# changzy00/pytorch-attention

Measured on AMD Instinct MI355X. Metric: forward images/sec through one step (+ ms/block), B=256 per GPU, 224x224-derived shapes, higher is better.
Workload: dtype f32/f16; 1 GPU; north-star step: C2 SE+CBAM+ECA, C3 ViT-Attn, C4 CSWin s1-4 + XCABlock + XCA, DA x2, Mixer, C5 ViT-Base fwd; B=256/GPU; precision=fp16-mfma, ranks_seen=1, gather=none (single rank), batch_per_gpu=256, parallelism=batch-shard x1, dist_backend=none, rccl_self_test=not run (single rank), distinct_gpus=1, full=off: --full adds calibration, roofline, per-block and CPU-baseline figures

## Files before the change

### include/mi355attn.h

```cpp
#ifndef MI355ATTN_H
#define MI355ATTN_H

#include <stddef.h>
#include <stdint.h>

#ifdef __cplusplus
extern "C" {
#endif

#define MI355_OK            0
#define MI355_EINVAL       -1
#define MI355_EUNSUPPORTED -2
#define MI355_EHIP         -3
#define MI355_ESYNC        -4
#define MI355_ERANGE (-5)

#define MI355_PREC_STRICT 0
#define MI355_PREC_FP16   1
#define MI355_PREC_BF16   2

#define MI355_ACT_NONE 0
#define MI355_ACT_GELU 1
#define MI355_ACT_RELU 2

// ... 88 lines not shown
};
size_t mi355_bam_workspace_bytes(int B, int C, int Cr, int H, int W);
int mi355_bam_fwd(const float* x, const float* const* params, float* y, int B, int C, int Cr, int H, int W, int dilation,
                  void* workspace, size_t workspace_bytes, mi355_stream_t stream);
int mi355_bam_gates_fwd(const float* x, const float* const* params, float* cg, float* sg, int B, int C, int Cr, int H, int W, int dilation,
                        void* workspace, size_t workspace_bytes, mi355_stream_t stream);
int mi355_zpool_fwd(const float* x, float* y, int B, int C, int H, int W, mi355_stream_t stream);
size_t mi355_attention_gate_workspace_bytes(int B, int H, int W);
int mi355_attention_gate_fwd(const float* x, const float* w, const float* affine, float* y, int B, int C, int H, int W, int ksize,
                             void* workspace, size_t workspace_bytes, mi355_stream_t stream);

enum {
    MI355_SK_CONV3_W = 0,
    MI355_SK_CONV3_SCALE,
    MI355_SK_CONV3_SHIFT,
    MI355_SK_CONV5_W,
    MI355_SK_CONV5_SCALE,
    MI355_SK_CONV5_SHIFT,
    MI355_SK_FC_W,
    MI355_SK_FC_B,
    MI355_SK_FC_BN_SCALE,
    MI355_SK_FC_BN_SHIFT,
    MI355_SK_FC1_W,
    MI355_SK_FC1_B,
    MI355_SK_FC2_W,
    MI355_SK_FC2_B,
    MI355_SK_NPARAMS
};
size_t mi355_sk_workspace_bytes(int B, int planes, int H, int W);
int mi355_sk_fwd(const float* x, const float* const* params, float* y, int B, int Cin, int planes, int groups, int d, int H, int W,
                 void* workspace, size_t workspace_bytes, mi355_stream_t stream);

size_t mi355_cam_workspace_bytes(int B, int C);
int mi355_cam_fwd(const float* x, const float* beta, float* y, int B, int C, int H, int W, int precision, void* workspace,
                  size_t workspace_bytes, mi355_stream_t stream);
int mi355_tokens_to_nchw_axpy_fwd(const float* tokens, const float* x, const float* alpha, float* y, int B, int HW, int C,
                                  mi355_stream_t stream);

int mi355_adaptive_pool_tokens_fwd(const float* x, float* y, int B, int H, int W, int C, int OH, int OW, mi355_stream_t stream);
int mi355_dwconv3x3_tokens_residual_fwd(const float* x, const float* weight, const float* bias, float* y, int B, int H, int W, int C,
                                        long y_batch_stride, mi355_stream_t stream);
int mi355_dwconv_nchw_tokens_fwd(const float* x, const float* weight, const float* bias, float* y, int B, int C, int H, int W, int ks,
                                 mi355_stream_t stream);
int mi355_qk_logits_fwd(const float* q, const float* k, float* logits, int B, int heads, int Nq, int Nkv, int head_dim, int ldq, int ldk,
                        int precision, mi355_stream_t stream);
int mi355_topk_mask_fwd(float* logits, long rows, int N, int k, mi355_stream_t stream);


int mi355_linear_fwd(const float* X, const float* W, const float* bias, const float* gamma, const float* resid,
                     float* Y, int M, int N, int K, int ldx, int ldy, int act, int precision,
                     mi355_stream_t stream);

int mi355_token_mix_fwd(const float* W, const float* X, const float* bias, const float* resid, float* Y,
                        int B, int T, int N, int C, int act, int precision, mi355_stream_t stream);

int mi355_layernorm_fwd(const float* x, const float* weight, const float* bias, float* y,
                        int rows, int cols, float eps, mi355_stream_t stream);

int mi355_cast16_fwd(const float* src, void* dst16, size_t n, int precision, mi355_stream_t stream);
int mi355_layernorm16_fwd(const float* x, const float* weight, const float* bias, void* y16, int rows, int cols, float eps,
                          int precision, mi355_stream_t stream);
int mi355_linear16_fwd(const void* X16, const void* W16, const float* bias, const float* gamma, const float* resid, void* Y,
                       int M, int N, int K, int ldx, int ldy, int act, int out16, int precision, mi355_stream_t stream);
size_t mi355_linear16_workspace_bytes(int M, int N, int K);
int mi355_linear16_x32_fwd(const float* X32, const void* W16, const float* bias, void* Y16, int M, int N, int K, int ldx, int ldy, int act,
                           int precision, mi355_stream_t stream);
int mi355_linear16_stats_fwd(const void* X16, const void* W16, const float* bias, const float* resid, float* Y, int M, int N, int K, int ldx,
                             int ldy, int precision, float* row_stats, float eps, mi355_stream_t stream);
int mi355_linear16_ln16_fwd(const void* X16, const void* W16, const float* bias, const float* resid, float* Y, const float* ln_w,
                            const float* ln_b, float eps, void* U16, int M, int N, int K, int ldx, int ldy, int ldu, int precision,
                            mi355_stream_t stream);
int mi355_linear16_ws_fwd(const void* X16, const void* W16, const float* bias, const float* gamma, const float* resid, void* Y,
                          int M, int N, int K, int ldx, int ldy, int act, int out16, int precision, void* ws, size_t ws_bytes,
                          mi355_stream_t stream);
int mi355_layernorm16_t_fwd(const float* x, const float* weight, const float* bias, void* ut16, int B, int N, int C, int NP, float eps,
                            int precision, mi355_stream_t stream);
int mi355_linear16_tr_fwd(const void* X16, const void* W16, const float* bias, const float* resid, float* Y, int M, int N, int K,
                          int ldx, int rows_per_image, int precision, mi355_stream_t stream);
size_t mi355_mixer_token_workspace_bytes(int B, int N, int C);
int mi355_mixer_token_fwd(const float* x, const float* ln_w, const float* ln_b, float ln_eps, const void* w1p16, const float* b1,
                          const void* w2s16, const float* b2, float* y, int B, int N, int C, int T, int precision, void* ws,
                          size_t ws_bytes, mi355_stream_t stream);
int mi355_ln_linear16_fwd(const float* X, const void* W16, const float* bias, void* Y, int M, int N, int K, int ldx, int ldy, float eps,
                          int act, int out16, int precision, mi355_stream_t stream);
int mi355_sdpa16_fwd(const void* qkv16, void* out16, int B, int N, int heads, int d, float scale, int precision,
                     mi355_stream_t stream);
int mi355_cswin_lepe_attn16_fwd(const void* qkv16, const float* getv_w, const float* getv_b, void* out16,
                                int B, int reso, int Ctot, int c0, int Cb, int heads, int Hsp, int Wsp,
                                float scale, int precision, mi355_stream_t stream);
int mi355_qkv_split16_fwd(const float* x, const void* w_hi, const void* w_lo, const void* w_v16, const float* bias, void* qkv5,
                          int M, int C, int K, int ldx, mi355_stream_t stream);
int mi355_sdpa16_split_fwd(const void* qkv5, void* out16, int B, int N, int heads, int d, float scale, mi355_stream_t stream);
int mi355_cswin_lepe_attn16_pair_fwd(const void* qkv16, const float* getv_w0, const float* getv_b0, const float* getv_w1,
                                     const float* getv_b1, void* out16, int B, int reso, int Ctot, int heads, int split, float scale,
                                     int precision, mi355_stream_t stream);

int mi355_proj_mlp_fused_fwd(const float* x, const void* ctx16, const void* wp16, const float* bp, const void* w1_16, const float* b1,
                             const void* w2_16, const float* b2, const float* gamma, float* y, long M, int C, int hidden, int layernorm,
                             float eps, int precision, mi355_stream_t stream);

int mi355_cswin_stripe_attn_fwd(const float* x, const void* wqkv16, const float* bqkv, const float* getv_w0, const float* getv_b0,
                                const float* getv_w1, const float* getv_b1, void* ctx16, int B, int reso, int C, int heads_per_branch,
                                int split, float scale, float eps, int precision, mi355_stream_t stream);

int mi355_mlp_fused_fwd(const float* x, const void* w1_16, const float* b1, const void* w2_16, const float* b2, const float* gamma,
                        float* y, long M, int C, int hidden, int layernorm, float eps, int precision, mi355_stream_t stream);


int mi355_sdpa_fwd(const float* qkv, float* out, int B, int N, int heads, int d, float scale, int precision,
                   mi355_stream_t stream);

int mi355_cswin_lepe_attn_fwd(const float* qkv, const float* getv_w, const float* getv_b, float* out,
                              int B, int reso, int Ctot, int c0, int Cb, int heads, int Hsp, int Wsp,
                              float scale, int precision, mi355_stream_t stream);

int mi355_xca_fwd(const float* qkv, const float* temperature, float* out, int B, int N, int heads, int d,
                  int precision, mi355_stream_t stream);
int mi355_xca16_fwd(const void* qkv, int qkv_is16, const float* temperature, void* out16, int B, int N, int heads, int d,
                    int precision, mi355_stream_t stream);

size_t mi355_lpi_workspace_bytes(int B, int H, int W, int C);
int    mi355_lpi_fwd(const float* x, const float* w1, const float* b1, const float* bn_w, const float* bn_b,
                     const float* bn_mean, const float* bn_var, float bn_eps, const float* w2, const float* b2,
                     const float* gamma, const float* resid, float* y, int B, int H, int W, int C,
                     void* ws, size_t ws_bytes, mi355_stream_t stream);
int    mi355_ln_lpi_fwd(const float* x, const float* ln_w, const float* ln_b, float ln_eps, const float* w1, const float* b1,
                        const float* bn_w, const float* bn_b, const float* bn_mean, const float* bn_var, float bn_eps, const float* w2,
                        const float* b2, const float* gamma, const float* resid, float* y, int B, int H, int W, int C, void* ws,
                        size_t ws_bytes, mi355_stream_t stream);

int mi355_patch_embed_fwd(const float* img, const float* Wp, const float* bp, const float* cls, const float* pos,
                          float* tokens, int B, int Cin, int H, int W, int ps, int E, int precision,
                          mi355_stream_t stream);
size_t mi355_patch_embed_workspace_bytes(int B, int Cin, int H, int W, int ps, int E, int precision);
int mi355_patch_embed_ws_fwd(const float* img, const float* Wp, const float* bp, const float* cls, const float* pos,
                             float* tokens, int B, int Cin, int H, int W, int ps, int E, int precision,
                             void* ws, size_t ws_bytes, mi355_stream_t stream);

size_t mi355_ln_fold_stats_bytes(int rows, int cols);
int mi355_ln_center16_fwd(const float* x, void* a16, float* rowtau, float* cvec, int rows, int cols, float eps, int precision,
                          mi355_stream_t stream);
int mi355_ln_finalize_fwd(const float* stats, const float* x, void* a16, float* cvec, float* rowtau, int rows, int cols, float eps,
                          float tol, int precision, unsigned* slow_rows, mi355_stream_t stream);
int mi355_linear16_emit_fwd(const void* X16, const void* W16, const float* bias, const float* resid, float* Y, int M, int N, int K, int ldx,
                            int act, int precision, const float* cvec, void* a16_out, float* stats, mi355_stream_t stream);
int mi355_linear16_lnfold_fwd(const void* A16, const void* W16, const float* bias, const float* rowtau, const float* colsum, void* Y16,
                              int M, int N, int K, int lda, int ldy, int act, int precision, mi355_stream_t stream);

size_t mi355_mhsa_workspace_bytes(int B, int N, int C, int x_is16);
int mi355_mhsa_fwd(const void* x, int x_is16, const void* Wqkv16, const float* b_qkv, const void* Wproj16, const float* b_proj,
                   const float* resid, float* y, int B, int N, int C, int heads, float scale, int precision, void* workspace,
                   size_t workspace_bytes, mi355_stream_t stream);

int mi355_sdpa_general_fwd(const void* q, const void* k, const void* v, const float* bias, void* out, int B, int num_heads, int Nq,
                           int Nkv, int head_dim, long ldq, long ldk, long ldv, long ldo, long bias_batch_stride, float scale,
                           int io16, int precision, mi355_stream_t stream);


int mi355_conv2d_tokens_fwd(const float* x, const float* weight, const float* bias, const float* pos, float* y, int B, int Cin,
                            int H, int W, int Cout, int KH, int KW, int stride, int pad, int ldw, int in_layout, int act,
                            int precision, mi355_stream_t stream);

int mi355_token_mean_fwd(const float* x, float* y, int B, int N, int C, long batch_stride, mi355_stream_t stream);

int mi355_class_attn_fwd(const float* q, const float* k, const float* v, float* out, int B, int N, int num_heads, int head_dim,
                         long ldq, long ldkv, float scale, mi355_stream_t stream);

int mi355_dwconv_patch_tokens_fwd(const float* x, const float* weight, const float* bias, float* y, int B, int H, int W, int C,
                                  int sr, mi355_stream_t stream);

int mi355_axpby_fwd(const float* x, const float* u, const float* gamma, float* y, long rows, int cols, long ldx, long ldu,
                    long ldy, float alpha, mi355_stream_t stream);

#define MI355_COMM_ID_BYTES 128
int    mi355_sdpa_core_fwd(const float* qkv, float* out, int B, int N, int heads, int d, float scale, int precision, mi355_stream_t stream);
size_t mi355_sdpa_core_workspace_bytes(int B, int N, int heads, int d);
int    mi355_gemm_bias_act_fwd(const float* X, const float* W, const float* bias, const float* gamma, const float* resid, float* Y, int M, int N,
                               int K, int ldx, int ldy, int act, int precision, mi355_stream_t stream);
size_t mi355_gemm_bias_act_workspace_bytes(int M, int N, int K);
int    mi355_mixer_token_mlp_fwd(const float* x, const float* ln_w, const float* ln_b, float ln_eps, const void* w1p16, const float* b1,
                                 const void* w2s16, const float* b2, float* y, int B, int N, int C, int T, int precision, void* ws,
                                 size_t ws_bytes, mi355_stream_t stream);
size_t mi355_mixer_token_mlp_workspace_bytes(int B, int N, int C);
size_t mi355_cswin_lepe_attn_workspace_bytes(int B, int reso, int Ctot);
size_t mi355_xca_workspace_bytes(int B, int N, int heads, int d);
size_t mi355_layernorm_workspace_bytes(int rows, int cols);

int mi355_ln_lpi_stats_fwd(const float* x, const float* stats, const float* ln_w, const float* ln_b, const float* w1, const float* b1,
                           const float* bn_w, const float* bn_b, const float* bn_mean, const float* bn_var, float bn_eps, const float* w2,
                           const float* b2, const float* gamma, const float* resid, float* y, int B, int H, int W, int C,
                           mi355_stream_t stream);

int mi355_comm_unique_id(void* id_out, size_t id_bytes);
int mi355_comm_init(const void* id, size_t id_bytes, int rank, int world, void** comm_out);
int mi355_allgather_f32(void* comm, const float* send, float* recv, size_t count, mi355_stream_t stream);
int mi355_comm_destroy(void* comm);

int mi355_bicubic_rows_fwd(const float* table, float* out, int n0h, int n0w, int oh, int ow, int dim, float scale_h, float scale_w,
                           mi355_stream_t stream);
int mi355_stream_copy(const void* src, void* dst, size_t bytes, mi355_stream_t stream);
int mi355_stream_read(const void* src, size_t bytes, float* sink, mi355_stream_t stream);
int mi355_mfma_yardstick(int shape, int iters, float* sink, unsigned long long* report, mi355_stream_t stream);
int mi355_event_time_begin(mi355_stream_t stream, void** handle);
int mi355_event_time_end(mi355_stream_t stream, void* handle, float* ms_out);

#ifdef __cplusplus
}
#endif
#endif
```

### pytorch-attention_amd/csrc/api.hip

```cpp
#include "common.h"
#include <atomic>
#include <cstring>
#include <mutex>
#include <algorithm>
#include <unordered_map>
#include <map>
#include <string>
#include <vector>

namespace mi355 {
static thread_local char g_err[512] = "";

constexpr int MAX_DEV = 64;
enum Opt { O_CHUNK_IMAGES, O_NT, O_REVERSE, O_GEMM_VARIANT, O_ECA_SINGLE, O_SE_SINGLE, O_CBAM_SINGLE, O_WS_PERSISTENT, O_STEM_DIRECT,
           O_ZOO_SINGLE, O_SPIN_LIMIT, O_GEMM_PA, O_GEMM_SPLITK, O_DA_FUSED, O_DA_RANGES, O_SE_OCC, O_LN_FOLD, O_GEMM_PA16, O_GEMM_PA_BLOCK, O_GEMM_PA_TAIL, O_LPI_PATCH, O_MIXER_FUSED, O_MIXER_EARLY, O_GEMM_SMALL, O_MLP_TT4, O_MIXER_STATS, O_ATTN_NW, O_GEMM_W4, O_RANGE_FALLBACK, O_GEMM_WREG, O_XCA_TR, O_MLP_WIDE, O_GEMM_WST, O_GEMM_WSLAB, O_IO16_OCC, O_COUNT };
struct OptDesc { const char* key; long def, lo, hi; };
static const OptDesc kOpts[O_COUNT] = {
    {"chunk_images", 0, 0, 1L << 40},
    {"nt", 3, 0, 3},
    {"reverse", 0, 0, 1},
    {"gemm_variant", 0, 0, 17},
    {"eca_single", 1, 0, 1},
    {"se_single", 1, 0, 1},
    {"cbam_single", 1, 0, 1},
    {"ws_persistent", 0, 0, 1},
    {"stem_direct", 1, 0, 1},
    {"zoo_single", 1, 0, 1},
    {"spin_limit", 1L << 22, 1024, 1L << 30},
    {"gemm_pa", 1, 0, 1},
    {"gemm_splitk", 1, 0, 1},
    {"da_fused", 1, 0, 1},
    {"da_ranges", 0, 0, 32},
    {"se_occ", 3, 2, 3},
    {"ln_fold", 0, 0, 1},
    {"gemm_pa16", 1, 0, 2},
    {"gemm_pa_block", 1, 0, 1},
    {"gemm_pa_tail", 10, 0, 100},
    {"lpi_patch", 1, 0, 1},
    {"mixer_fused", 1, 0, 1},
    {"mixer_early", 0, 0, 1},
    {"gemm_small", 1, 0, 1},
    {"mlp_tt4", 0, 0, 1},
    {"mixer_stats", 0, 0, 1},
    {"attn_nw", 8, 7, 8},
    {"gemm_w4", 1, 0, 1},
    {"range_fallback", 1, 0, 1},
    {"gemm_wreg", 1, 0, 1},
    {"xca_tr", 1, 0, 1},
    {"mlp_wide", 0, 0, 1},
    {"gemm_wst", 0, 0, 4},
    {"gemm_wslab", 1, 0, 2},
    {"io16_occ", 4, 2, 4},
};
static_assert(sizeof(kOpts) / sizeof(kOpts[0]) == O_COUNT, "one table row per option, in enum order");
namespace {
constexpr long OPT_UNSET = (long)0x8000000000000000ull;
struct OptBlock { std::atomic<long> v[O_COUNT]; };
OptBlock g_opt[MAX_DEV];
std::atomic<long> g_def[O_COUNT];
std::once_flag g_opt_once;
int cur_dev() {
    int dev = 0;
    if (hipGetDevice(&dev) != hipSuccess) { (void)hipGetLastError(); dev = 0; }
    return dev >= 0 && dev < MAX_DEV ? dev : 0;
}
void opt_init() {
    std::call_once(g_opt_once, [] {
        for (int i = 0; i < O_COUNT; ++i) g_def[i].store(kOpts[i].def, std::memory_order_relaxed);
        for (auto& b : g_opt)
            for (int i = 0; i < O_COUNT; ++i) b.v[i].store(OPT_UNSET, std::memory_order_relaxed);
    });
}
inline long opt(Opt o) {
    opt_init();
    const long v = g_opt[cur_dev()].v[o].load(std::memory_order_relaxed);
    return v != OPT_UNSET ? v : g_def[o].load(std::memory_order_relaxed);
}
}

char* err_buf() { return g_err; }

int fail(int code, const char* fmt, ...) {
    va_list ap;
    va_start(ap, fmt);
    vsnprintf(g_err, sizeof(g_err), fmt, ap);
    va_end(ap);
    return code;
}
long opt_chunk_images() { return opt(O_CHUNK_IMAGES); }
long opt_nt() { return opt(O_NT); }
long opt_reverse() { return opt(O_REVERSE); }
long opt_eca_single() { return opt(O_ECA_SINGLE); }
long opt_se_single() { return opt(O_SE_SINGLE); }
long opt_cbam_single() { return opt(O_CBAM_SINGLE); }
long opt_ws_persistent() { return opt(O_WS_PERSISTENT); }
long opt_ln_fold() { return opt(O_LN_FOLD); }
long opt_gemm_pa16() { return opt(O_GEMM_PA16); }
long opt_gemm_pa_block() { return opt(O_GEMM_PA_BLOCK); }
long opt_gemm_pa_tail() { return opt(O_GEMM_PA_TAIL); }
long opt_lpi_patch() { return opt(O_LPI_PATCH); }
long opt_mixer_early() { return opt(O_MIXER_EARLY); }
long opt_gemm_small() { return opt(O_GEMM_SMALL); }
long opt_mlp_tt4() { return opt(O_MLP_TT4); }
long opt_mixer_stats() { return opt(O_MIXER_STATS); }
long opt_attn_nw() { return opt(O_ATTN_NW); }
long opt_gemm_w4() { return opt(O_GEMM_W4); }
long opt_range_fallback() { return opt(O_RANGE_FALLBACK); }
long opt_gemm_wreg() { return opt(O_GEMM_WREG); }
long opt_xca_tr() { return opt(O_XCA_TR); }
long opt_mlp_wide() { return opt(O_MLP_WIDE); }
long opt_gemm_wst() { return opt(O_GEMM_WST); }
long opt_gemm_wslab() { return opt(O_GEMM_WSLAB); }

namespace {
struct WsEntry { unsigned long long key; };
std::mutex g_ws_mu;
std::unordered_map<const void*, WsEntry> g_ws;
}

bool stream_is_capturing(hipStream_t st) {
    hipStreamCaptureStatus cs = hipStreamCaptureStatusNone;
    if (hipStreamIsCapturing(st, &cs) != hipSuccess) {
        (void)hipGetLastError();
        return false;
    }
    return cs != hipStreamCaptureStatusNone;
}

bool ws_known(const void* region, unsigned long long key, hipStream_t st) {
    if (!opt_ws_persistent()) return false;
    std::lock_guard<std::mutex> lk(g_ws_mu);
    auto it = g_ws.find(region);
    if (it != g_ws.end() && it->second.key == key) return true;
    if (!stream_is_capturing(st)) g_ws[region] = WsEntry{key};
    return false;
}
namespace {
__global__ __launch_bounds__(256) void ws_zero_kernel(unsigned* p, size_t words) {
    for (size_t i = (size_t)blockIdx.x * 256 + threadIdx.x; i < words; i += (size_t)gridDim.x * 256) p[i] = 0u;
}
}
hipError_t ws_zero_async(void* p, size_t bytes, hipStream_t st) {
    const size_t words = bytes / 4;
    if (!words) return hipSuccess;
    size_t blocks = (words + 1023) / 1024;
    if (blocks > 2048) blocks = 2048;
    ws_zero_kernel<<<(int)blocks, 256, 0, st>>>(static_cast<unsigned*>(p), words);
    return hipGetLastError();
}
void ws_forget(const void* region) {
    std::lock_guard<std::mutex> lk(g_ws_mu);
    g_ws.erase(region);
}
void ws_forget_range(const void* base, size_t bytes) {
    std::lock_guard<std::mutex> lk(g_ws_mu);
    const char* lo = static_cast<const char*>(base);
    for (auto it = g_ws.begin(); it != g_ws.end();) {
        const char* p = static_cast<const char*>(it->first);
        if (p >= lo && p < lo + bytes) it = g_ws.erase(it);
        else ++it;
    }
}

namespace {
constexpr int THREAD_SLOTS = 64;
constexpr size_t SLOT_WORDS = 16 * MAX_DEV;
std::once_flag g_sync_once;
unsigned* g_sync_block = nullptr;
std::mutex g_slot_mu;
bool g_slot_used[THREAD_SLOTS] = {};
struct ThreadSlot {
    int idx = -1;
    ~ThreadSlot() {
        if (idx < 0 || idx >= THREAD_SLOTS) return;
        std::lock_guard<std::mutex> lk(g_slot_mu);
        g_slot_used[idx] = false;
    }
};
thread_local ThreadSlot t_slot;
unsigned* thread_words() {
    if (!g_sync_block) return nullptr;
    if (t_slot.idx < 0) {
        std::lock_guard<std::mutex> lk(g_slot_mu);
        int i = 0;
        while (i < THREAD_SLOTS && g_slot_used[i]) ++i;
        if (i < THREAD_SLOTS) {
            g_slot_used[i] = true;
            std::memset(g_sync_block + i * SLOT_WORDS, 0, SLOT_WORDS * sizeof(unsigned));
        }
        t_slot.idx = i;
    }
    return g_sync_block + t_slot.idx * SLOT_WORDS + 16 * cur_dev();
}
}
unsigned* sync_err_word() {
    std::call_once(g_sync_once, [] {
        const size_t bytes = (THREAD_SLOTS + 1) * SLOT_WORDS * sizeof(unsigned);
        void* p = nullptr;
        if (hipHostMalloc(&p, bytes, hipHostMallocMapped | hipHostMallocCoherent | hipHostMallocPortable) == hipSuccess && p) {
            std::memset(p, 0, bytes);
            g_sync_block = static_cast<unsigned*>(p);
        } else {
            (void)hipGetLastError();
        }
    });
    return thread_words();
}
unsigned* sync_err_word_on(hipStream_t st) {
    if (!g_sync_block && stream_is_capturing(st)) return nullptr;
    return sync_err_word();
}
namespace {
struct RangeMark {
    int armed = 0, dirty = 0, fresh = 0, have = 0, count = 0, expect = 0;
    hipEvent_t ev = nullptr;
    hipStream_t st = nullptr;
};
std::mutex g_ev_mu;
std::vector<hipEvent_t> g_ev_pool[MAX_DEV];
struct ThreadMarks {
    RangeMark m[MAX_DEV];
    ~ThreadMarks() {
        std::lock_guard<std::mutex> lk(g_ev_mu);
        for (int d = 0; d < MAX_DEV; ++d)
            if (m[d].ev) g_ev_pool[d].push_back(m[d].ev);
    }
};
thread_local ThreadMarks t_marks;
RangeMark& rmark(int dev) { return t_marks.m[dev]; }
void range_mark_record(RangeMark& m, int dev) {
    m.dirty = 0;
    if (stream_is_capturing(m.st)) return;
    if (!m.ev) {
        {
            std::lock_guard<std::mutex> lk(g_ev_mu);
            if (!g_ev_pool[dev].empty()) { m.ev = g_ev_pool[dev].back(); g_ev_pool[dev].pop_back(); }
        }
        if (!m.ev && hipEventCreateWithFlags(&m.ev, hipEventDisableTiming) != hipSuccess) { (void)hipGetLastError(); m.ev = nullptr; return; }
    }
    if (hipEventRecord(m.ev, m.st) == hipSuccess) m.have = 1;
    else (void)hipGetLastError();
}
}
void range_mark_before_launch() {
    const int dev = cur_dev();
    RangeMark& m = rmark(dev);
    if (!m.dirty || m.fresh) return;
    if (m.expect > 0 && m.count >= m.expect) range_mark_record(m, dev);
}
void range_mark_entry_done() {
    RangeMark& m = rmark(cur_dev());
    if (!m.fresh) return;
    m.fresh = 0;
    m.dirty = 1;
}
unsigned* range_word(hipStream_t st) {
    if (!g_sync_block && stream_is_capturing(st)) return nullptr;
    unsigned* w = sync_err_word();
    if (w) {
        RangeMark& m = rmark(cur_dev());
        if (m.armed) {
            m.st = st;
            ++m.count;
            m.fresh = 1;
        }
// ... 277 lines not shown
```

### pytorch-attention_amd/csrc/attn.hip

```cpp
#include "common.h"
#include "mma.h"
#include "bufops.h"
#include <type_traits>

namespace {

struct AttnArgs {
    const void* qkv;
    void* out;
    const float* lepe_w;
    const float* lepe_b;
    int L, Ctot, c0, heads;
    int koff, voff, oc0;
    int reso, Hsp, Wsp, nWx, nwin;
    int T;
    unsigned wsp_magic;
    float scale;
    int pre_scale;
};

struct AttnPair {
    AttnArgs a0, a1;
    int split;
};
struct AttnPairRg : AttnPair {
    unsigned* ovf;
};
template <bool IO16>
using attn_kargs = typename std::conditional<IO16, AttnPair, AttnPairRg>::type;
template <bool IO16>
const attn_kargs<IO16>& attn_pick(const AttnPairRg& p) { return p; }

#ifndef MI355_ATTN_FMA_SM
#define MI355_ATTN_FMA_SM 1
#endif
template <int PREC, int D, int KT, bool LEPE, bool IO16, int NW, int OCC = 1, int TFULL = -1>
__global__ __launch_bounds__(NW * 64, OCC) void win_attn_kernel(const attn_kargs<IO16> pr) {
    constexpr bool FMA_SM = MI355_ATTN_FMA_SM != 0;
    const int lid = xcd_contiguous_block();
    const bool second = lid >= pr.split;
    const AttnArgs a = second ? pr.a1 : pr.a0;
    constexpr int NTHR = NW * 64;
    static_assert(!IO16 || PREC != 0, "16-bit I/O exists for the fp16 / bf16 operand modes only");
    using M_ = Mma<PREC>;
    using v8 = typename M_::v8;
    using v4 = typename M_::v4;
    using el = typename M_::e;
    constexpr int NS = M_::NSPLIT;
    constexpr int TK = KT * 16;
    constexpr int KP = D + 8;
    constexpr int VP = TK + 4;
    constexpr bool RG = !IO16 && PREC == 1;
    float rgm = 0.f;
    constexpr int OP = IO16 ? D + 8 : D + 4;
    constexpr int K_EL = TK * KP, V_EL = D * VP;
    using slab_t = typename std::conditional<IO16, unsigned short, float>::type;
    __shared__ __attribute__((aligned(16))) unsigned short s_k[NS * K_EL];
    __shared__ __attribute__((aligned(16))) unsigned short s_v[NS * V_EL];
    __shared__ __attribute__((aligned(16))) slab_t s_o[NW * 16 * OP];

    const int t = threadIdx.x, lane = t & 63, wave = t >> 6;
    int bid = lid - (second ? pr.split : 0);
    const int head = bid % a.heads; bid /= a.heads;
    const int win = bid % a.nwin;
    const int b = bid / a.nwin;
    const int T = a.T;
    const int wy0 = (win / a.nWx) * a.Hsp, wx0 = (win % a.nWx) * a.Wsp;
    const int ch0 = a.c0 + head * D;
    const int och0 = a.oc0 + head * D;
    const long row3 = 3L * a.Ctot;
    using gel = typename std::conditional<IO16, el, float>::type;
    const gel* base = static_cast<const gel*>(a.qkv) + (long)b * a.L * row3 + ch0;
    auto srow = [&](int s) { return a.Wsp == 1 ? s : (int)__umulhi((unsigned)s, a.wsp_magic); };
    auto tok = [&](int s) { const int r = srow(s); return (wy0 + r) * a.reso + wx0 + (s - r * a.Wsp); };

    const int l15 = lane & 15, g = lane >> 4;
    const int nqt = (T + 15) >> 4;
    constexpr int NQ = (KT + NW - 1) / NW;
    const rsrc_t img_rs = make_rsrc(IO16 ? static_cast<const void*>(base) : nullptr, IO16 ? (bufops_u32)((long)a.L * row3 * sizeof(gel)) : 0u);
    auto ld16 = [&](bool live, int token, int el_off) -> v8 {
        const bufops_u32 off = live ? (bufops_u32)((token * (int)row3 + el_off) * 2) : OOB;
        return __builtin_bit_cast(v8, __builtin_amdgcn_raw_buffer_load_b128(img_rs, off, 0, 0));
    };
    v8 qraw[IO16 ? NQ : 1][D / 32];
    if constexpr (IO16) {
#pragma unroll
        for (int iq = 0; iq < NQ; ++iq) {
            const int qs = (wave + iq * NW) * 16 + l15;
            const int tq = tok(qs < T ? qs : 0);
#pragma unroll
            for (int ks = 0; ks < D / 32; ++ks) qraw[iq][ks] = ld16(qs < T, tq, ks * 32 + g * 8);
        }
    }
    __shared__ float s_lw[LEPE ? D * 10 : 1];
    if constexpr (LEPE) {
        for (int q = t; q < D * 10; q += NTHR) {
            const int c = q / 10, i = q - c * 10;
            s_lw[q] = i < 9 ? a.lepe_w[(long)(head * D + c) * 9 + i] : a.lepe_b[head * D + c];
        }
    }

    constexpr int D4 = D / 4;
    if constexpr (IO16) {
        constexpr int D8 = D / 8;
        constexpr int NKI = (TK * D8 + NTHR - 1) / NTHR, NVI = ((TK / 4) * D8 + NTHR - 1) / NTHR;
        v8 kreg[NKI];
        v8 vreg[NVI][4];
#pragma unroll
        for (int it = 0; it < NKI; ++it) {
            const int idx = t + it * NTHR, key = idx / D8, d8 = idx % D8;
            const bool live = idx < TK * D8 && key < T;
            kreg[it] = ld16(live, tok(live ? key : 0), a.koff + d8 * 8);
        }
#pragma unroll
        for (int it = 0; it < NVI; ++it) {
            const int idx = t + it * NTHR, kg = idx / D8, d8 = idx % D8;
#pragma unroll
            for (int j = 0; j < 4; ++j) {
                const int key = kg * 4 + j;
                const bool live = idx < (TK / 4) * D8 && key < T;
                vreg[it][j] = ld16(live, tok(live ? key : 0), a.voff + d8 * 8);
            }
        }
#pragma unroll
        for (int it = 0; it < NKI; ++it) {
            const int idx = t + it * NTHR, key = idx / D8, d8 = idx % D8;
            if (idx < TK * D8) *reinterpret_cast<v8*>(s_k + key * KP + d8 * 8) = kreg[it];
        }
#pragma unroll
        for (int it = 0; it < NVI; ++it) {
            const int idx = t + it * NTHR, kg = idx / D8, d8 = idx % D8;
            if (idx < (TK / 4) * D8) {
#pragma unroll
                for (int q = 0; q < 8; ++q)
                    *reinterpret_cast<v4*>(s_v + (d8 * 8 + q) * VP + kg * 4) =
                        v4{vreg[it][0][q], vreg[it][1][q], vreg[it][2][q], vreg[it][3][q]};
            }
        }
    } else {
    for (int idx = t; idx < TK * D4; idx += NTHR) {
        const int key = idx / D4, d4 = idx % D4;
        f4 v = {0.f, 0.f, 0.f, 0.f};
        if (key < T) v = *reinterpret_cast<const f4*>(base + (long)tok(key) * row3 + a.koff + d4 * 4);
        if constexpr (RG) rgm = rg_absmax4(rgm, v);
        const v4 h = M_::cvt(v);
        *reinterpret_cast<v4*>(s_k + key * KP + d4 * 4) = h;
        if constexpr (NS == 2) *reinterpret_cast<v4*>(s_k + K_EL + key * KP + d4 * 4) = M_::cvt_lo(v, h);
    }
    for (int idx = t; idx < (TK / 4) * D4; idx += NTHR) {
        const int kg = idx / D4, d4 = idx % D4;
        f4 r[4];
#pragma unroll
        for (int j = 0; j < 4; ++j) {
            const int key = kg * 4 + j;
            r[j] = f4{0.f, 0.f, 0.f, 0.f};
            if (key < T) r[j] = *reinterpret_cast<const f4*>(base + (long)tok(key) * row3 + a.voff + d4 * 4);
            if constexpr (RG) rgm = rg_absmax4(rgm, r[j]);
        }
        const f4 c[4] = {{r[0].x, r[1].x, r[2].x, r[3].x}, {r[0].y, r[1].y, r[2].y, r[3].y},
                         {r[0].z, r[1].z, r[2].z, r[3].z}, {r[0].w, r[1].w, r[2].w, r[3].w}};
#pragma unroll
        for (int q = 0; q < 4; ++q) {
            const v4 h = M_::cvt(c[q]);
            *reinterpret_cast<v4*>(s_v + (d4 * 4 + q) * VP + kg * 4) = h;
            if constexpr (NS == 2) *reinterpret_cast<v4*>(s_v + V_EL + (d4 * 4 + q) * VP + kg * 4) = M_::cvt_lo(c[q], h);
        }
    }
    }
    __shared__ unsigned short s_tap[LEPE ? TK * 9 : 1];
    if constexpr (LEPE) {
        for (int q = t; q < NS * D; q += NTHR) s_v[(q / D) * V_EL + (q % D) * VP + TK] = 0;
        for (int q = t; q < T * 9; q += NTHR) {
            const int slot = q / 9, tap = q - slot * 9;
            const int ty = srow(slot), tx = slot - ty * a.Wsp;
            const int yy = ty + tap / 3 - 1, xx = tx + tap % 3 - 1;
            s_tap[q] = (unsigned short)(((yy >= 0 && yy < a.Hsp && xx >= 0 && xx < a.Wsp) ? yy * a.Wsp + xx : TK) * 2);
        }
    }
    __syncthreads();

    slab_t* slab = s_o + wave * 16 * OP;
#pragma unroll
    for (int iq = 0; iq < NQ; ++iq) {
        const int qt = wave + iq * NW;
        if (qt >= nqt) break;
        const int qs = qt * 16 + l15;
        v8 qf[D / 32][NS];
        {
            const gel* qrow = base + (long)tok(qs < T ? qs : 0) * row3;
#pragma unroll
            for (int ks = 0; ks < D / 32; ++ks) {
                f4 lo4 = {0.f, 0.f, 0.f, 0.f}, hi4 = {0.f, 0.f, 0.f, 0.f};
                if constexpr (IO16) {
                    const v8 raw = qraw[iq][ks];
                    if (!a.pre_scale) { qf[ks][0] = raw; continue; }
                    lo4 = f4{(float)raw[0], (float)raw[1], (float)raw[2], (float)raw[3]};
                    hi4 = f4{(float)raw[4], (float)raw[5], (float)raw[6], (float)raw[7]};
                } else if (qs < T) {
                    lo4 = *reinterpret_cast<const f4*>(qrow + ks * 32 + g * 8);
                    hi4 = *reinterpret_cast<const f4*>(qrow + ks * 32 + g * 8 + 4);
                }
                if (a.pre_scale) { lo4 = lo4 * a.scale; hi4 = hi4 * a.scale; }
                if constexpr (RG) rgm = rg_absmax4(rg_absmax4(rgm, lo4), hi4);
                const v4 h0 = M_::cvt(lo4), h1 = M_::cvt(hi4);
                qf[ks][0] = v8{h0.x, h0.y, h0.z, h0.w, h1.x, h1.y, h1.z, h1.w};
                if constexpr (NS == 2) {
                    const v4 e0 = M_::cvt_lo(lo4, h0), e1 = M_::cvt_lo(hi4, h1);
                    qf[ks][1] = v8{e0.x, e0.y, e0.z, e0.w, e1.x, e1.y, e1.z, e1.w};
                }
            }
        }
        f4 o[D / 16];
        float sum;
        const f4 zero4 = {0.f, 0.f, 0.f, 0.f};
        f4 s[KT];
#pragma unroll
        for (int kt = 0; kt < KT; ++kt) {
            f4 acc = zero4;
            if (kt < TFULL || kt * 16 < T) {
#pragma unroll
                for (int ks = 0; ks < D / 32; ++ks) {
                    v8 kf[NS];
#pragma unroll
                    for (int sp = 0; sp < NS; ++sp)
                        kf[sp] = *reinterpret_cast<const v8*>(s_k + sp * K_EL + (kt * 16 + l15) * KP + ks * 32 + g * 8);
                    acc = mma_step<PREC>(kf, qf[ks], acc);
                }
            }
            s[kt] = acc;
        }
        const float post = (a.pre_scale ? 1.0f : a.scale) * 1.44269504088896340736f;
        float m = -INFINITY;
        sum = 0.f;
        if constexpr (PREC != 0 && FMA_SM) {
#pragma unroll
            for (int kt = 0; kt < KT; ++kt)
#pragma unroll
                for (int r = 0; r < 4; ++r) {
                    const int key = kt * 16 + g * 4 + r;
                    const float v = (kt < TFULL || key < T) ? s[kt][r] : -INFINITY;
                    s[kt][r] = v;
                    m = fmaxf(m, v);
                }
            m = fmaxf(m, __shfl_xor(m, 16, WAVE));
            m = fmaxf(m, __shfl_xor(m, 32, WAVE));
            const float mneg = -(m * post);
#pragma unroll
            for (int kt = 0; kt < KT; ++kt)
#pragma unroll
                for (int r = 0; r < 4; ++r) {
                    s[kt][r] = __builtin_amdgcn_exp2f(__builtin_fmaf(s[kt][r], post, mneg));
                }
        } else {
#pragma unroll
            for (int kt = 0; kt < KT; ++kt)
#pragma unroll
                for (int r = 0; r < 4; ++r) {
                    const int key = kt * 16 + g * 4 + r;
                    const float v = (kt < TFULL || key < T) ? s[kt][r] * post : -INFINITY;
                    s[kt][r] = v;
                    m = fmaxf(m, v);
                }
            m = fmaxf(m, __shfl_xor(m, 16, WAVE));
            m = fmaxf(m, __shfl_xor(m, 32, WAVE));
#pragma unroll
            for (int kt = 0; kt < KT; ++kt)
#pragma unroll
                for (int r = 0; r < 4; ++r) {
                    const float p = __builtin_amdgcn_exp2f(s[kt][r] - m);
                    s[kt][r] = p;
                    sum += p;
                }
        }
        if constexpr (!(PREC != 0 && FMA_SM)) {
            sum += __shfl_xor(sum, 16, WAVE);
            sum += __shfl_xor(sum, 32, WAVE);
        }
#pragma unroll
        for (int nt = 0; nt < D / 16; ++nt) o[nt] = zero4;
        f4 osum = zero4;
        typedef typename M_::e el1_t;
        const v8 ones = v8{(el1_t)1.0f, (el1_t)1.0f, (el1_t)1.0f, (el1_t)1.0f, (el1_t)1.0f, (el1_t)1.0f, (el1_t)1.0f, (el1_t)1.0f};
#pragma unroll
        for (int kb = 0; kb < KT / 2; ++kb) {
            if (2 * kb < TFULL || kb * 32 < T) {
                v8 pf[NS];
                {
                    const f4 p0 = s[2 * kb], p1 = s[2 * kb + 1];
                    const v4 h0 = M_::cvt(p0), h1 = M_::cvt(p1);
                    pf[0] = v8{h0.x, h0.y, h0.z, h0.w, h1.x, h1.y, h1.z, h1.w};
                    if constexpr (NS == 2) {
                        const v4 e0 = M_::cvt_lo(p0, h0), e1 = M_::cvt_lo(p1, h1);
                        pf[1] = v8{e0.x, e0.y, e0.z, e0.w, e1.x, e1.y, e1.z, e1.w};
                    }
                }
#pragma unroll
                for (int nt = 0; nt < D / 16; ++nt) {
                    v8 vf[NS];
#pragma unroll
                    for (int sp = 0; sp < NS; ++sp) {
                        const unsigned short* vr = s_v + sp * V_EL + (nt * 16 + l15) * VP + kb * 32 + g * 4;
                        const v4 a0 = *reinterpret_cast<const v4*>(vr);
                        const v4 a1 = *reinterpret_cast<const v4*>(vr + 16);
                        vf[sp] = v8{a0.x, a0.y, a0.z, a0.w, a1.x, a1.y, a1.z, a1.w};
                    }
                    o[nt] = mma_step<PREC>(vf, pf, o[nt]);
                }
                if constexpr (PREC != 0 && FMA_SM) osum = M_::mma(ones, pf[0], osum);
            }
        }
        if constexpr (PREC != 0 && FMA_SM) sum = osum.x;
        const float inv = __builtin_amdgcn_rcpf(sum);
        int off[LEPE ? 9 : 1];
        bool qlive = false;
        if constexpr (LEPE) {
            const int qslot = qt * 16 + l15;
            qlive = qslot < T;
            const unsigned short* tp = s_tap + (qlive ? qslot : 0) * 9;
#pragma unroll
            for (int i = 0; i < 9; ++i) off[i] = tp[i];
        }
#pragma unroll
        for (int nt = 0; nt < D / 16; ++nt) {
            f4 val = o[nt] * inv;
            if constexpr (LEPE) {
                if (qlive) {
#pragma unroll
                    for (int r = 0; r < 4; ++r) {
                        const int d = nt * 16 + g * 4 + r;
                        const float* lwp = s_lw + d * 10;
                        const char* vrow = reinterpret_cast<const char*>(s_v + d * VP);
                        float acc = lwp[9];
#pragma unroll
                        for (int i = 0; i < 9; ++i) {
                            float vv = (float)(*reinterpret_cast<const el*>(vrow + off[i]));
                            if constexpr (NS == 2) vv += (float)(*reinterpret_cast<const el*>(vrow + V_EL * 2 + off[i]));
                            acc = __builtin_fmaf(lwp[i], vv, acc);
                        }
                        val[r] += acc;
                    }
                }
            }
            if constexpr (IO16) *reinterpret_cast<v4*>(slab + l15 * OP + nt * 16 + g * 4) = M_::cvt(val);
            else *reinterpret_cast<f4*>(slab + l15 * OP + nt * 16 + g * 4) = val;
        }
        __builtin_amdgcn_wave_barrier();
        __builtin_amdgcn_fence(__ATOMIC_ACQ_REL, "wavefront");
        if constexpr (IO16) {
            constexpr int LPR = D / 8, RPI = 64 / LPR;
#pragma unroll
            for (int it = 0; it < 16 / RPI; ++it) {
                const int r = it * RPI + lane / LPR, c8 = (lane % LPR) * 8;
                const int qslot = qt * 16 + r;
                if (qslot < T)
                    *reinterpret_cast<v8*>(static_cast<gel*>(a.out) + ((long)b * a.L + tok(qslot)) * a.Ctot + och0 + c8) =
                        *reinterpret_cast<const v8*>(slab + r * OP + c8);
            }
        } else {
            constexpr int LPR = D / 4, RPI = 64 / LPR;
#pragma unroll
            for (int it = 0; it < 16 / RPI; ++it) {
                const int r = it * RPI + lane / LPR, c4 = (lane % LPR) * 4;
                const int qslot = qt * 16 + r;
                if (qslot < T)
                    *reinterpret_cast<f4*>(static_cast<gel*>(a.out) + ((long)b * a.L + tok(qslot)) * a.Ctot + och0 + c4) =
                        *reinterpret_cast<const f4*>(slab + r * OP + c4);
            }
        }
        __builtin_amdgcn_wave_barrier();
        __builtin_amdgcn_fence(__ATOMIC_ACQ_REL, "wavefront");
    }
    if constexpr (RG) rg_report(rgm, pr.ovf, 7u);
}

template <int D, bool LEPE, bool IO16>
int launch_attn(const AttnArgs& a, int B, int precision, hipStream_t st, const AttnArgs* other = nullptr) {
    AttnPairRg pr{};
    pr.a0 = a;
    pr.split = B * a.nwin * a.heads;
    int grid = pr.split;
    if (other) {
        pr.a1 = *other;
        grid += B * other->nwin * other->heads;
    }
    if (IO16 && precision == MI355_PREC_STRICT)
        return mi355::fail(MI355_EINVAL, "16-bit activation I/O needs precision 1 (fp16) or 2 (bf16)");
    if (!IO16 && precision == MI355_PREC_FP16) pr.ovf = mi355::range_word(st);
    MI355_TRACE(st, "win_attn_kernel<d=%d%s%s> B=%d windows=%d heads=%d tokens=%d", D, LEPE ? ",lepe" : "", IO16 ? ",io16" : "", B, a.nwin, a.heads, a.T);
#define GO(P, KT_, NW_) win_attn_kernel<P, D, KT_, LEPE, (IO16 && P != 0), NW_><<<grid, NW_ * 64, 0, st>>>(attn_pick<(IO16 && P != 0)>(pr))
#define GO_OCC(P, KT_, NW_, OCC_) win_attn_kernel<P, D, KT_, LEPE, (IO16 && P != 0), NW_, ((IO16 && P != 0 && D == 32) ? OCC_ : 1)><<<grid, NW_ * 64, 0, st>>>(attn_pick<(IO16 && P != 0)>(pr))
#define GO_FULL(P, KT_, NW_, OCC_, TF_) \
    win_attn_kernel<P, D, KT_, LEPE, (IO16 && P != 0), NW_, ((IO16 && P != 0 && D == 32) ? OCC_ : 1), TF_><<<grid, NW_ * 64, 0, st>>>(attn_pick<(IO16 && P != 0)>(pr))
    const bool hot = IO16 && (!other || other->T == a.T);
#define BYKT(P)                                          \
    do {                                                 \
        if (a.T <= 64) { if (hot && P != 0 && a.T >= 48) GO_FULL(P, 4, 4, 6, 3); else GO_OCC(P, 4, 4, 6); }          \
        else if (a.T <= 128) { if (hot && P != 0 && a.T >= 96) GO_FULL(P, 8, 4, 5, 6); else GO_OCC(P, 8, 4, 5); }    \
        else if (IO16 && P != 0) {                                                                                    \
             \
                                \
            if (a.T >= 192 && a.T <= 208 && mi355::opt_attn_nw() == 7) GO_FULL(P, 14, 7, 1, 12);                          \
            else if (a.T >= 192) GO_FULL(P, 14, 8, 1, 12); else GO(P, 14, 8); }                                          \
        else GO(P, 14, 4);                               \
    } while (0)
    switch (precision) {
        case MI355_PREC_STRICT: BYKT(0); break;
        case MI355_PREC_FP16:   BYKT(1); break;
        case MI355_PREC_BF16:   BYKT(2); break;
        default: return mi355::fail(MI355_EINVAL, "precision must be 0, 1 or 2 (got %d)", precision);
    }
#undef BYKT
#undef GO_FULL
#undef GO_OCC
#undef GO
    return MI355_OK;
}

}

static int sdpa_common(const void* qkv, void* out, int B, int N, int heads, int d, float scale, int precision, bool io16,
                       hipStream_t st) {
    AttnArgs a{};
    a.qkv = qkv; a.out = out; a.L = N; a.Ctot = heads * d; a.c0 = 0; a.heads = heads;
    a.koff = a.Ctot; a.voff = 2 * a.Ctot; a.oc0 = 0;
    a.reso = N; a.Hsp = 1; a.Wsp = N; a.nWx = 1; a.nwin = 1; a.T = N; a.scale = scale; a.pre_scale = 0;
    a.wsp_magic = (unsigned)(((1ull << 32) + (unsigned)N - 1) / (unsigned)N);
    if (d == 64) return io16 ? launch_attn<64, false, true>(a, B, precision, st) : launch_attn<64, false, false>(a, B, precision, st);
    return io16 ? launch_attn<32, false, true>(a, B, precision, st) : launch_attn<32, false, false>(a, B, precision, st);
}

static AttnArgs lepe_args(const void* qkv, const float* getv_w, const float* getv_b, void* out, int reso, int Ctot, int c0, int heads,
                          int Hsp, int Wsp, float scale) {
    AttnArgs a{};
    a.qkv = qkv; a.out = out; a.lepe_w = getv_w; a.lepe_b = getv_b;
    a.L = reso * reso; a.Ctot = Ctot; a.c0 = c0; a.heads = heads;
    a.koff = Ctot; a.voff = 2 * Ctot; a.oc0 = c0;
    a.reso = reso; a.Hsp = Hsp; a.Wsp = Wsp; a.nWx = reso / Wsp; a.nwin = (reso / Hsp) * (reso / Wsp); a.T = Hsp * Wsp;
    a.scale = scale; a.pre_scale = 1;
    a.wsp_magic = (unsigned)(((1ull << 32) + (unsigned)Wsp - 1) / (unsigned)Wsp);
    return a;
}

static int lepe_common(const void* qkv, const float* getv_w, const float* getv_b, void* out, int B, int reso, int Ctot, int c0, int Cb,
                       int heads, int Hsp, int Wsp, float scale, int precision, bool io16, hipStream_t st) {
    (void)Cb;
    const AttnArgs a = lepe_args(qkv, getv_w, getv_b, out, reso, Ctot, c0, heads, Hsp, Wsp, scale);
    return io16 ? launch_attn<32, true, true>(a, B, precision, st) : launch_attn<32, true, false>(a, B, precision, st);
}

#define SDPA_CHECKS(fn)                                                                                                   \
    MI355_CHECK_ARG(qkv && out && B > 0 && N > 0 && heads > 0);                                                           \
    if (!(d == 32 || d == 64)) return mi355::fail(MI355_EUNSUPPORTED, fn ": head dim %d (built: 32, 64)", d);            \
    if (N > 224) return mi355::fail(MI355_EUNSUPPORTED, fn ": sequence length %d > 224 (single-pass softmax core)", N);   \
    MI355_CHECK_ARG(aligned16(qkv) && aligned16(out))

#define LEPE_CHECKS(fn)                                                                                                    \
    MI355_CHECK_ARG(qkv && getv_w && getv_b && out);                                                                       \
    MI355_CHECK_ARG(B > 0 && reso > 0 && Ctot > 0 && c0 >= 0 && Cb > 0 && c0 + Cb <= Ctot && heads > 0 && Cb % heads == 0); \
    MI355_CHECK_ARG(Hsp > 0 && Wsp > 0 && reso % Hsp == 0 && reso % Wsp == 0);                                             \
    if (Cb / heads != 32) return mi355::fail(MI355_EUNSUPPORTED, fn ": head dim %d (built: 32)", Cb / heads);             \
    if (Hsp * Wsp > 224) return mi355::fail(MI355_EUNSUPPORTED, fn ": %d tokens per stripe window > 224", Hsp * Wsp);     \
    MI355_CHECK_ARG((Ctot & 7) == 0 && (c0 & 7) == 0 && aligned16(qkv) && aligned16(out))

extern "C" {

int mi355_sdpa_fwd(const float* qkv, float* out, int B, int N, int heads, int d, float scale, int precision,
                   mi355_stream_t stream) {
    SDPA_CHECKS("mi355_sdpa_fwd");
    int rc = sdpa_common(qkv, out, B, N, heads, d, scale, precision, false, static_cast<hipStream_t>(stream));
    if (rc) return rc;
    MI355_LAUNCH_CHECK();
    return MI355_OK;
}

int mi355_sdpa16_fwd(const void* qkv, void* out, int B, int N, int heads, int d, float scale, int precision,
                     mi355_stream_t stream) {
    SDPA_CHECKS("mi355_sdpa16_fwd");
    int rc = sdpa_common(qkv, out, B, N, heads, d, scale, precision, true, static_cast<hipStream_t>(stream));
    if (rc) return rc;
    MI355_LAUNCH_CHECK();
    return MI355_OK;
}

int mi355_cswin_lepe_attn_fwd(const float* qkv, const float* getv_w, const float* getv_b, float* out, int B, int reso, int Ctot,
                              int c0, int Cb, int heads, int Hsp, int Wsp, float scale, int precision, mi355_stream_t stream) {
    LEPE_CHECKS("mi355_cswin_lepe_attn_fwd");
    int rc = lepe_common(qkv, getv_w, getv_b, out, B, reso, Ctot, c0, Cb, heads, Hsp, Wsp, scale, precision, false,
                         static_cast<hipStream_t>(stream));
    if (rc) return rc;
    MI355_LAUNCH_CHECK();
    return MI355_OK;
}

int mi355_cswin_lepe_attn16_pair_fwd(const void* qkv, const float* getv_w0, const float* getv_b0, const float* getv_w1, const float* getv_b1,
                                     void* out, int B, int reso, int Ctot, int heads, int split, float scale, int precision,
                                     mi355_stream_t stream) {
    MI355_CHECK_ARG(qkv && getv_w0 && getv_b0 && getv_w1 && getv_b1 && out);
    MI355_CHECK_ARG(B > 0 && reso > 0 && Ctot > 0 && heads > 0 && (Ctot / 2) % heads == 0 && split > 0 && reso % split == 0);
    if (Ctot / 2 / heads != 32) return mi355::fail(MI355_EUNSUPPORTED, "mi355_cswin_lepe_attn16_pair_fwd: head dim %d (built: 32)", Ctot / 2 / heads);
    if (reso * split > 224) return mi355::fail(MI355_EUNSUPPORTED, "mi355_cswin_lepe_attn16_pair_fwd: %d tokens per stripe window > 224", reso * split);
    MI355_CHECK_ARG((Ctot & 15) == 0 && aligned16(qkv) && aligned16(out));
    const AttnArgs a0 = lepe_args(qkv, getv_w0, getv_b0, out, reso, Ctot, 0, heads, reso, split, scale);
    const AttnArgs a1 = lepe_args(qkv, getv_w1, getv_b1, out, reso, Ctot, Ctot / 2, heads, split, reso, scale);
    int rc = launch_attn<32, true, true>(a0, B, precision, static_cast<hipStream_t>(stream), &a1);
    if (rc) return rc;
    MI355_LAUNCH_CHECK();
    return MI355_OK;
}

int mi355_cswin_lepe_attn16_fwd(const void* qkv, const float* getv_w, const float* getv_b, void* out, int B, int reso, int Ctot,
                                int c0, int Cb, int heads, int Hsp, int Wsp, float scale, int precision, mi355_stream_t stream) {
    LEPE_CHECKS("mi355_cswin_lepe_attn16_fwd");
    int rc = lepe_common(qkv, getv_w, getv_b, out, B, reso, Ctot, c0, Cb, heads, Hsp, Wsp, scale, precision, true,
                         static_cast<hipStream_t>(stream));
    if (rc) return rc;
    MI355_LAUNCH_CHECK();
    return MI355_OK;
}

}
```

### pytorch-attention_amd/csrc/common.h

```cpp
#pragma once
#include <hip/hip_runtime.h>
#include <cstdarg>
#include <cstdio>
#include <cstdint>
#include "../../include/mi355attn.h"

#define MI355_ABI_VERSION 1
#define WAVE 64

namespace mi355 {
char* err_buf();
int   fail(int code, const char* fmt, ...);
long  opt_chunk_images();
long  opt_nt();
long  opt_reverse();
long  opt_gemm_variant();
long  opt_gemm_splitk();
long  opt_gemm_pa();
long  opt_da_fused();
long  opt_da_ranges();
long  opt_eca_single();
long  opt_se_single();
long  opt_se_occ();
long  opt_io16_occ();
long  opt_ws_persistent();
long  opt_ln_fold();
long  opt_gemm_pa16();
long  opt_gemm_pa_block();
long  opt_gemm_pa_tail();
long  opt_lpi_patch();
long  opt_mixer_early();
long  opt_gemm_small();
long  opt_mlp_tt4();
long  opt_mixer_stats();
long  opt_attn_nw();
long  opt_gemm_w4();
long  opt_gemm_wreg();
long  opt_xca_tr();
long  opt_mlp_wide();
long  opt_gemm_wst();
long  opt_gemm_wslab();
bool  mlp_wide_applicable(int C, int hidden);
int   mlp_wide(const float* x, const void* w1_16, const float* b1, const void* w2_16, const float* b2, const float* gamma, float* y, long M, int C,
               int layernorm, float eps, int precision, hipStream_t st);
int   gemm_small_nt(const float* A, const float* B, const float* bias, float* C, int M, int N, int K, int lda, int ldb, int ldc, int precision,
                    hipStream_t st);
void  ws_forget(const void* region);
bool  ws_known(const void* region, unsigned long long key, hipStream_t st);
hipError_t ws_zero_async(void* p, size_t bytes, hipStream_t st);
unsigned* sync_err_word_on(hipStream_t st);
bool  stream_is_capturing(hipStream_t st);
void  ws_forget_range(const void* base, size_t bytes);
long  opt_cbam_single();
unsigned* sync_err_word();
unsigned* range_word(hipStream_t st);
int   range_pending(const char* who);
void  range_mark_before_launch();
void  range_mark_entry_done();
int   range_arm(int on);
int   range_wait();
long  range_launches();
unsigned  spin_limit();
int   sync_pending(const char* who);
int   resident_slots(int per_cu);
bool  trace_on();
int   trace_begin();
long  trace_end(char* buf, size_t n);
struct TraceScope {
    int idx;
    hipStream_t st;
    TraceScope(hipStream_t st_, const char* fmt, ...);
    ~TraceScope();
    TraceScope(const TraceScope&) = delete;
    TraceScope& operator=(const TraceScope&) = delete;
};
#define MI355_TRACE(st, ...) mi355::TraceScope trace_scope_(st, __VA_ARGS__)
int   func_dynamic_lds(const void* fn, int bytes);
long  opt_zoo_single();
long  opt_stem_direct();
bool  stem_conv_applicable(int Cin, int Cout, int KH, int KW, int in_layout, const float* bias, const float* pos, const float* y);
int   stem_conv(const float* x, const float* w, const float* bias, const float* pos, float* y, int B, int Cin, int H, int W, int Cout, int KH,
                int KW, int stride, int pad, int ldw, int in_layout, int act, hipStream_t st);
size_t zoo_workspace_bytes(int B, int C);
size_t cbam_single_extra_bytes(int B, int C, int H, int W);
bool  cbam_single_applicable(int C, int Cr, int H, int W, int ks);
int   cbam_single(const float* x, const float* w1, const float* w2, const float* wconv, float* y, int B, int C, int Cr, int H, int W,
                  int ks, void* extra, hipStream_t st);
size_t se_single_extra_bytes(int B, int C);
bool  se_single_applicable(int C, int Cr, int H, int W);
struct SeExtra {
    const float* b1;
    const float* b2;
    int gate;
};
int   se_single(const float* x, const float* w1, const float* w2, float* y, int B, int C, int Cr, int H, int W, void* state,
                void* gran, SeExtra ex, hipStream_t st);
bool  eca_single_applicable(int C, int k, int H, int W);
int   eca_single(const float* x, const float* taps, float* y, int B, int C, int k, int H, int W, hipStream_t st);
size_t fused_state_bytes(int B);
bool   double_attn_fused_ok(int B, int C, int cm, int cn, int HW, int precision);
size_t double_attn_fused_workspace(int B, int C, int HW);
int    double_attn_fused(const float* x, const float* wA, const float* bA, const float* wB, const float* bB, const float* wV, const float* bV,
                         const float* wP, const float* bP, float* y, int B, int C, int HW, int precision, void* ws, hipStream_t st);
bool   double_attn_small_ok(int B, int C, int cm, int cn, int HW, int precision);
int    double_attn_small(const float* x, const float* wA, const float* bA, const float* wB, const float* bB, const float* wV, const float* bV,
                         const float* wP, const float* bP, float* y, int B, int C, int HW, int precision, hipStream_t st);
int gemm_nt(const float* A, const float* B, const float* bias, const float* gamma, const float* resid, float* C, int M, int N,
            int K, int lda, int ldb, int ldc, int act, int precision, hipStream_t st);
int gemm_nt_batched(const float* A, const float* B, float* C, int batch, int M, int N, int K, int lda, int ldb, int ldc, long sA,
                    long sB, long sC, int precision, hipStream_t st);
int gemm_kn_batched(const float* A, const float* B, const float* bias_row, const float* resid, float* C, int batch, int M,
                    int N, int K, int lda, int ldb, int ldc, long sA, long sB, long sC, int act, int precision,
                    hipStream_t st);
}

#define MI355_CHECK_ARG(cond)                                                                   \
    do {                                                                                        \
        if (!(cond)) return mi355::fail(MI355_EINVAL, "%s: invalid argument: %s", __func__, #cond); \
    } while (0)

#define MI355_HIP(call)                                                                         \
    do {                                                                                        \
        hipError_t e_ = (call);                                                                 \
        if (e_ != hipSuccess)                                                                   \
            return mi355::fail(MI355_EHIP, "%s: %s -> %s", __func__, #call, hipGetErrorString(e_)); \
    } while (0)

#define MI355_LAUNCH_CHECK()                                                                    \
    do {                                                                                        \
        hipError_t e_ = hipGetLastError();                                                      \
        if (e_ != hipSuccess)                                                                   \
            return mi355::fail(MI355_EHIP, "%s: kernel launch -> %s", __func__, hipGetErrorString(e_)); \
        mi355::range_mark_entry_done();                                                         \
    } while (0)

static inline bool aligned16(const void* p) { return (reinterpret_cast<uintptr_t>(p) & 15u) == 0; }
static inline int  cdiv(long a, long b) { return (int)((a + b - 1) / b); }

#if defined(__HIPCC__)
__device__ __forceinline__ float wave_sum(float v) {
#pragma unroll
    for (int o = 32; o > 0; o >>= 1) v += __shfl_xor(v, o, WAVE);
    return v;
}
__device__ __forceinline__ float wave_max(float v) {
#pragma unroll
    for (int o = 32; o > 0; o >>= 1) v = fmaxf(v, __shfl_xor(v, o, WAVE));
    return v;
}
template <int XOR> __device__ __forceinline__ float swz_xor(float v) {
    return __builtin_bit_cast(float, __builtin_amdgcn_ds_swizzle(__builtin_bit_cast(int, v), (XOR << 10) | 0x1f));
}
__device__ __forceinline__ float wave_sum_sw(float v) {
    float a = v, b = v;
    asm volatile("s_nop 1\n\tv_permlane32_swap_b32 %0, %1\n\ts_nop 1" : "+v"(a), "+v"(b));
    v = a + b;
    v += swz_xor<16>(v);
    v += swz_xor<8>(v);
    v += swz_xor<4>(v);
    v += swz_xor<2>(v);
    v += swz_xor<1>(v);
    return v;
}

__device__ __forceinline__ int xcd_contiguous_block() {
    const int nwg = gridDim.x, orig = blockIdx.x, xcd = orig & 7, q = nwg >> 3, r = nwg & 7;
    return (xcd < r ? xcd * (q + 1) : r * (q + 1) + (xcd - r) * q) + (orig >> 3);
}
__device__ __forceinline__ float relu_nan(float v) {
    const float r = fmaxf(v, 0.f);
    return ((__float_as_uint(v) & 0x7fffffffu) > 0x7f800000u) ? v : r;
}
__device__ __forceinline__ float sigmoidf_(float z) { return 1.0f / (1.0f + expf(-z)); }
typedef float rg_f4 __attribute__((ext_vector_type(4)));
__device__ __forceinline__ float rg_fold(float m, float g) {
    const int u = (int)(__float_as_uint(g) + 0x00800000u);
    const int mi = (int)__float_as_uint(m);
    return __uint_as_float((unsigned)(u > mi ? u : mi));
}
__device__ __forceinline__ float rg_absmax4(float m, rg_f4 v) {
    return rg_fold(m, fmaxf(fmaxf(fabsf(v.x), fabsf(v.y)), fmaxf(fabsf(v.z), fabsf(v.w))));
}
__device__ __forceinline__ float rg_absmax1(float m, float v) { return rg_fold(m, fabsf(v)); }
__device__ __forceinline__ void rg_report(float m, unsigned* word, unsigned code) {
    if (word && (int)__float_as_uint(m) >= (int)(0x477FF000u + 0x00800000u))
        __hip_atomic_store(word, code, __ATOMIC_RELAXED, __HIP_MEMORY_SCOPE_SYSTEM);
}
__device__ __forceinline__ float rg_absmax4_f(float m, rg_f4 v) {
    const float g = fmaxf(fmaxf(fabsf(v.x), fabsf(v.y)), fmaxf(fabsf(v.z), fabsf(v.w)));
    return g < __builtin_inff() ? fmaxf(m, g) : m;
}
__device__ __forceinline__ void rg_report_f(float m, unsigned* word, unsigned code) {
    if (word && m >= 65520.0f) __hip_atomic_store(word, code, __ATOMIC_RELAXED, __HIP_MEMORY_SCOPE_SYSTEM);
}
// ... 85 lines not shown
```

### pytorch-attention_amd/csrc/gemm16.h

```cpp
#pragma once
#include "common.h"
#include "mma.h"

namespace g16 {

constexpr int BK = 64;

struct G16Args {
    const void* A; const void* B; void* C;
    const float* bias; const float* gamma; const float* resid;
    int M, N, K, lda, ldb, ldc;
    int act;
    int tr_rows;
    int resid_period;
    unsigned* ovf;
    const float* Af;
    float ln_eps;
    void* lnc_a; int lnc_lda; float* lnc_stats; const float* lnc_c;
    const float* rowtau; const float* colsum;
    float* row_stats;
    void* ln16_out; const float* ln16_w; const float* ln16_b; int ln16_ld;
};

template <typename T> struct Vec8;
template <> struct Vec8<_Float16> { using t = h8; using t4 = h4; };
template <> struct Vec8<__bf16> { using t = b8; using t4 = b4; };

template <typename T>
__device__ __forceinline__ f4 mma16(typename Vec8<T>::t a, typename Vec8<T>::t b, f4 c);
template <>
__device__ __forceinline__ f4 mma16<_Float16>(h8 a, h8 b, f4 c) { return __builtin_amdgcn_mfma_f32_16x16x32_f16(a, b, c, 0, 0, 0); }
template <>
__device__ __forceinline__ f4 mma16<__bf16>(b8 a, b8 b, f4 c) { return __builtin_amdgcn_mfma_f32_16x16x32_bf16(a, b, c, 0, 0, 0); }

}

namespace mi355 {
int gemm16_p8(const g16::G16Args& g, int out16, int precision, void* ws, size_t ws_bytes, hipStream_t st);
size_t gemm16_p8_workspace_bytes(int M, int N, int K);
int gemm16_pa(const g16::G16Args& g, int out16, int precision, hipStream_t st, int abl = 0);
int gemm16_w4(const g16::G16Args& g, int out16, int precision, hipStream_t st);
int gemm16_wreg(const g16::G16Args& g, int out16, int precision, hipStream_t st);
int gemm16_wst(const g16::G16Args& g, int out16, int precision, hipStream_t st);
int gemm16_wslab(const g16::G16Args& g, int out16, int precision, hipStream_t st);
int gemm16_wslab_check(const g16::G16Args& g, int precision);
int linear16_dispatch(const g16::G16Args& g, int out16, int precision, void* ws, size_t ws_bytes, hipStream_t st);
}
```

### pytorch-attention_amd/csrc/gemm16.hip

```cpp
#include <type_traits>
#include "gemm16.h"

namespace {
using namespace g16;

template <typename T, bool OUT16, int BM, int BN, int WM, int WN, bool PRIO, int STAGES, bool TR = false>
__global__ __launch_bounds__(WM * WN * 64) void gemm16_kernel(const G16Args g) {
    using v8 = typename Vec8<T>::t;
    using v4 = typename Vec8<T>::t4;
    constexpr int NW = WM * WN;
    constexpr int TM = BM / WM, TN = BN / WN, MF = TM / 16, NF = TN / 16;
    constexpr int STAGE = (BM + BN) * BK;
    constexpr int IA = BM / 8 / NW, IB = BN / 8 / NW;
    constexpr int LDS_BYTES = STAGES * STAGE * 2;
    static_assert(BM % (8 * NW) == 0 && BN % (8 * NW) == 0 && TM % 32 == 0 && TN % 16 == 0, "tile/wave geometry");
    __shared__ __attribute__((aligned(16))) unsigned char lds_raw[LDS_BYTES];
    T* lds = reinterpret_cast<T*>(lds_raw);

    const int t = threadIdx.x, lane = t & 63, wave = t >> 6;
    const int wr = wave / WN, wc = wave % WN;
    const int tiles_n = (g.N + BN - 1) / BN;
    int wg;
    {
        const int nwg = gridDim.x, bid = blockIdx.x, xcd = bid & 7, q = nwg >> 3, r = nwg & 7;
// ... 439 lines not shown
    const int rc2 = mi355::gemm16_wslab(g, 1, precision, st);
    if (rc2 != MI355_OK) return rc2;
    MI355_LAUNCH_CHECK();
    return MI355_OK;
}

int mi355_linear16_ws_fwd(const void* X16, const void* W16, const float* bias, const float* gamma, const float* resid, void* Y, int M,
                          int N, int K, int ldx, int ldy, int act, int out16, int precision, void* ws, size_t ws_bytes,
                          mi355_stream_t stream) {
    MI355_CHECK_ARG(X16 && W16 && Y && M > 0 && N > 0 && K > 0 && ldx >= K && ldy >= N);
    MI355_CHECK_ARG(act == MI355_ACT_NONE || act == MI355_ACT_GELU);
    MI355_CHECK_ARG(precision == MI355_PREC_FP16 || precision == MI355_PREC_BF16);
    if ((K % BK) || (N & 3) || (ldx & 7) || (ldy & 3) || !aligned16(X16) || !aligned16(W16) || !aligned16(Y) ||
        (bias && !aligned16(bias)) || (gamma && !aligned16(gamma)) || (resid && !aligned16(resid)))
        return mi355::fail(MI355_EUNSUPPORTED, "mi355_linear16_fwd: needs K %% 64 == 0, N %% 4 == 0, 16-byte aligned rows (K=%d N=%d ldx=%d)",
                           K, N, ldx);
    G16Args g{};
    g.A = X16; g.B = W16; g.C = Y; g.bias = bias; g.gamma = gamma; g.resid = resid;
    g.M = M; g.N = N; g.K = K; g.lda = ldx; g.ldb = K; g.ldc = ldy; g.act = act;
    if (out16 && precision == MI355_PREC_FP16) g.ovf = mi355::range_word(static_cast<hipStream_t>(stream));
    return mi355::linear16_dispatch(g, out16, precision, ws, ws_bytes, static_cast<hipStream_t>(stream));
}

int mi355_linear16_stats_fwd(const void* X16, const void* W16, const float* bias, const float* resid, float* Y, int M, int N, int K, int ldx,
                             int ldy, int precision, float* row_stats, float eps, mi355_stream_t stream) {
    MI355_CHECK_ARG(X16 && W16 && resid && Y && row_stats && M > 0 && N > 0 && K > 0 && ldx >= K && ldy >= N);
    MI355_CHECK_ARG(precision == MI355_PREC_FP16 || precision == MI355_PREC_BF16);
    G16Args g{};
    g.row_stats = row_stats; g.ln_eps = eps;
    if (const int rc = linear16_wreg_fwd(g, X16, W16, bias, resid, Y, M, N, K, ldx, ldy, precision, static_cast<hipStream_t>(stream),
                                         "mi355_linear16_stats_fwd", "and a statistics pass"))
        return rc;
    MI355_LAUNCH_CHECK();
    return MI355_OK;
}

int mi355_linear16_ln16_fwd(const void* X16, const void* W16, const float* bias, const float* resid, float* Y, const float* ln_w,
                            const float* ln_b, float eps, void* U16, int M, int N, int K, int ldx, int ldy, int ldu, int precision,
                            mi355_stream_t stream) {
    MI355_CHECK_ARG(X16 && W16 && resid && Y && ln_w && ln_b && U16 && M > 0 && N > 0 && K > 0 && ldx >= K && ldy >= N && ldu >= N);
    MI355_CHECK_ARG(precision == MI355_PREC_FP16 || precision == MI355_PREC_BF16);
    G16Args g{};
    g.ln16_out = U16; g.ln16_w = ln_w; g.ln16_b = ln_b; g.ln16_ld = ldu; g.ln_eps = eps;
    if (const int rc = linear16_wreg_fwd(g, X16, W16, bias, resid, Y, M, N, K, ldx, ldy, precision, static_cast<hipStream_t>(stream),
                                         "mi355_linear16_ln16_fwd", "+ mi355_layernorm16_fwd"))
        return rc;
    MI355_LAUNCH_CHECK();
    return MI355_OK;
}

}

int mi355::linear16_dispatch(const G16Args& g, int out16, int precision, void* ws, size_t ws_bytes, hipStream_t st) {
    const int M = g.M, N = g.N, K = g.K;
    if (g.resid_period && (K == 64 || K == 128 || out16 || !g.resid)) return MI355_EUNSUPPORTED;
    const struct { long variant, wst, wslab, pa, pa16, pa_tail, wreg, w4; } opt = {
        mi355::opt_gemm_variant(), mi355::opt_gemm_wst(), mi355::opt_gemm_wslab(), mi355::opt_gemm_pa(), mi355::opt_gemm_pa16(),
        mi355::opt_gemm_pa_tail(), mi355::opt_gemm_wreg(), mi355::opt_gemm_w4()};
    const int ncu = mi355::resident_slots(1);
    const bool gelu = g.act == MI355_ACT_GELU;
    long variant = opt.variant;
    if (variant >= 15) {
        static const char* const what[] = {"persistent kernel",
                                           "the two-accumulator kernel",
                                           "the one-wave-per-SIMD kernel"};
        const int rc = variant == 15 ? mi355::gemm16_p8(g, out16, precision, ws, ws_bytes, st)
                     : variant == 16 ? mi355::gemm16_pa(g, out16, precision, st) : mi355::gemm16_w4(g, out16, precision, st);
        if (rc == MI355_EUNSUPPORTED) return mi355::fail(rc, "mi355_linear16_fwd: %s does not take this shape", what[variant - 15]);
        return checked(rc);
    }
    if (variant == 0) {
        int rc;
        if ((opt.wst == 2 || opt.wst == 4 || ((opt.wst & 1) && g.act == MI355_ACT_NONE)) &&
            (rc = checked(mi355::gemm16_wst(g, out16, precision, st))) != MI355_EUNSUPPORTED)
            return rc;
        if ((K == 64 || K == 128) && M >= 2048 && (!out16 || (N & 7) == 0)) {
            MI355_TRACE(st, "gemm16_ws_kernel<%s> M=%d N=%d K=%d", out16 ? "out16" : "out32", M, N, K);
            launch_ws<false>(g, out16, precision, K == 64 ? 2 : 1, ncu, st);
            MI355_LAUNCH_CHECK();
            return MI355_OK;
        }
        if ((opt.wslab == 2 || (opt.wslab == 1 && (gelu || (M & 255)))) &&
            (rc = checked(mi355::gemm16_wslab(g, out16, precision, st))) != MI355_EUNSUPPORTED)
            return rc;
        const long pa_tiles = (N & 255) ? (long)(M / 256) * (N / 128) : (long)cdiv(M, 128) * (N / 256);
        const bool pa_fills = 2 * pa_tiles >= ncu;
        if (out16 && opt.pa && pa_fills && (K <= 512 || (opt.pa16 >= 1 && gelu) || opt.pa16 >= 2) &&
            (rc = checked(mi355::gemm16_pa(g, out16, precision, st))) != MI355_EUNSUPPORTED)
            return rc;
        if (opt.wreg && (rc = checked(mi355::gemm16_wreg(g, out16, precision, st))) != MI355_EUNSUPPORTED) return rc;
        if (!out16 && (g.resid || N <= 768) && opt.pa && pa_fills) {
            const int bmt = (N & 255) ? 256 : 128, tn = (N & 255) ? N / 128 : N / 256;
            const long left = pa_tiles % ncu;
            if (opt.pa_tail > 0 && pa_tiles > ncu && left > 0 && left * 100 <= opt.pa_tail * ncu && K >= 1024 && M % bmt == 0 &&
                !g.resid_period && !g.lnc_a) {
                const int rows1 = (int)((pa_tiles - left) / tn) * bmt, rows2 = M - rows1;
                G16Args g1 = g, g2 = g;
                g1.M = rows1;
                g2.M = rows2;
                g2.A = static_cast<const char*>(g.A) + (size_t)rows1 * g.lda * 2;
                g2.C = static_cast<char*>(g.C) + (size_t)rows1 * g.ldc * 4;
                if (g.resid) g2.resid = g.resid + (size_t)rows1 * g.ldc;
                rc = mi355::gemm16_pa(g1, out16, precision, st);
                if (rc == MI355_OK) {
                    MI355_LAUNCH_CHECK();
                    const int grid = cdiv(rows2, 32) * cdiv(N, 64);
                    MI355_TRACE(st, "gemm16_kernel<tail 32x64> M=%d N=%d K=%d", rows2, N, K);
                    if (precision == MI355_PREC_FP16) gemm16_kernel<_Float16, false, 32, 64, 1, 4, false, 10><<<grid, 256, 0, st>>>(g2);
                    else                              gemm16_kernel<__bf16, false, 32, 64, 1, 4, false, 10><<<grid, 256, 0, st>>>(g2);
                    MI355_LAUNCH_CHECK();
                    return MI355_OK;
                }
                if (rc != MI355_EUNSUPPORTED) return rc;
            }
            if ((rc = checked(mi355::gemm16_pa(g, out16, precision, st))) != MI355_EUNSUPPORTED) return rc;
        }
        if ((long)cdiv(M, 256) * cdiv(N, 256) >= ncu && K >= 256) {
            if (out16 && K >= 576 && K < 1536 && opt.w4 && (rc = checked(mi355::gemm16_w4(g, out16, precision, st))) != MI355_EUNSUPPORTED)
                return rc;
            if ((rc = checked(mi355::gemm16_p8(g, out16, precision, ws, ws_bytes, st))) != MI355_EUNSUPPORTED) return rc;
        }
        variant = (N <= 64) ? 9 : (N < 256 ? 1 : 7);
        if (variant == 7 && (long)cdiv(M, 128) * cdiv(N, 256) < ncu) variant = 1;
    }
    else if (variant == 8) variant = 0;
    MI355_TRACE(st, "gemm16_kernel<variant %ld,%s> M=%d N=%d K=%d%s", variant, out16 ? "out16" : "out32", M, N, K, gelu ? " gelu" : "");
#define LAUNCH(T_, O_, BM_, BN_, WM_, WN_, P_, S_)                                                         \
    gemm16_kernel<T_, O_, BM_, BN_, WM_, WN_, P_, S_><<<cdiv(M, BM_) * cdiv(N, BN_), WM_ * WN_ * 64, 0, st>>>(g)
#define BY_VARIANT(T_, O_)                                                 \
    do {                                                                   \
        switch (variant) {                                                 \
            case 1: LAUNCH(T_, O_, 128, 128, 2, 2, true, 2); break;        \
            case 2: LAUNCH(T_, O_, 256, 128, 4, 2, false, 2); break;       \
            case 3: LAUNCH(T_, O_, 256, 256, 2, 4, false, 2); break;       \
            case 4: LAUNCH(T_, O_, 256, 256, 2, 4, true, 2); break;        \
            case 5: LAUNCH(T_, O_, 128, 128, 2, 2, true, 1); break;        \
            case 6: LAUNCH(T_, O_, 256, 128, 4, 2, true, 1); break;        \
            case 7: LAUNCH(T_, O_, 128, 256, 2, 4, true, 1); break;        \
            case 9: LAUNCH(T_, O_, 256, 64, 4, 1, true, 1); break;         \
            default: LAUNCH(T_, O_, 128, 128, 2, 2, false, 2); break;      \
        }                                                                  \
    } while (0)
    if (precision == MI355_PREC_FP16) {
        if (out16) BY_VARIANT(_Float16, true); else BY_VARIANT(_Float16, false);
    } else {
        if (out16) BY_VARIANT(__bf16, true); else BY_VARIANT(__bf16, false);
    }
#undef BY_VARIANT
#undef LAUNCH
    MI355_LAUNCH_CHECK();
    return MI355_OK;
}

extern "C" {

int mi355_linear16_tr_fwd(const void* X16, const void* W16, const float* bias, const float* resid, float* Y, int M, int N, int K,
                          int ldx, int rows_per_image, int precision, mi355_stream_t stream) {
    MI355_CHECK_ARG(X16 && W16 && Y && M > 0 && N > 0 && K > 0 && ldx >= K && rows_per_image > 0);
    MI355_CHECK_ARG(precision == MI355_PREC_FP16 || precision == MI355_PREC_BF16);
    if ((K % BK) || (ldx & 7) || (rows_per_image & 3) || (M % rows_per_image) || !aligned16(X16) || !aligned16(W16) || !aligned16(Y) ||
        (resid && !aligned16(resid)))
        return mi355::fail(MI355_EUNSUPPORTED, "mi355_linear16_tr_fwd: needs K %% 64 == 0, rows_per_image %% 4 == 0 dividing M (K=%d M=%d rows=%d)",
                           K, M, rows_per_image);
    G16Args g{};
    g.A = X16; g.B = W16; g.C = Y; g.bias = bias; g.resid = resid;
    g.M = M; g.N = N; g.K = K; g.lda = ldx; g.ldb = K; g.ldc = N; g.act = MI355_ACT_NONE; g.tr_rows = rows_per_image;
    hipStream_t st = static_cast<hipStream_t>(stream);
    const bool wide = N > 128 && ((N & 255) == 0 || (N & 127) != 0);
    MI355_TRACE(st, "gemm16_kernel<transposed out> M=%d N=%d K=%d", M, N, K);
#define TRL(T_, BN_, WN_) gemm16_kernel<T_, false, 128, BN_, 2, WN_, true, 1, true><<<cdiv(M, 128) * cdiv(N, BN_), 2 * WN_ * 64, 0, st>>>(g)
    if (precision == MI355_PREC_FP16) { if (wide) TRL(_Float16, 256, 4); else TRL(_Float16, 128, 2); }
    else                              { if (wide) TRL(__bf16, 256, 4); else TRL(__bf16, 128, 2); }
#undef TRL
    MI355_LAUNCH_CHECK();
    return MI355_OK;
}

int mi355_ln_linear16_fwd(const float* X, const void* W16, const float* bias, void* Y, int M, int N, int K, int ldx, int ldy, float eps,
                          int act, int out16, int precision, mi355_stream_t stream) {
    MI355_CHECK_ARG(X && W16 && Y && M > 0 && N > 0 && ldx >= K && ldy >= N);
    MI355_CHECK_ARG(act == MI355_ACT_NONE || act == MI355_ACT_GELU);
    MI355_CHECK_ARG(precision == MI355_PREC_FP16 || precision == MI355_PREC_BF16);
    if (!(K == 64 || K == 128) || (N & 7) || (ldx & 3) || (ldy & 7) || !aligned16(X) || !aligned16(W16) || !aligned16(Y) || (bias && !aligned16(bias)))
        return mi355::fail(MI355_EUNSUPPORTED, "mi355_ln_linear16_fwd: built for K = 64 / 128, N %% 8 == 0, 16-byte aligned rows (K=%d N=%d)", K, N);
    G16Args g{};
    g.Af = X; g.B = W16; g.C = Y; g.bias = bias; g.ln_eps = eps;
    g.M = M; g.N = N; g.K = K; g.lda = ldx; g.ldb = K; g.ldc = ldy; g.act = act;
    hipStream_t st = static_cast<hipStream_t>(stream);
    if (out16 && precision == MI355_PREC_FP16) g.ovf = mi355::range_word(st);
    const int ncu = mi355::resident_slots(1);
    MI355_TRACE(st, "gemm16_ws_kernel<ln,%s> M=%d N=%d K=%d", out16 ? "out16" : "out32", M, N, K);
    launch_ws<true>(g, out16, precision, 2, ncu, st);
    MI355_LAUNCH_CHECK();
    return MI355_OK;
}

}
```

### pytorch-attention_amd/csrc/layernorm.hip

```cpp
#include "common.h"
#include "mma.h"
#include <type_traits>

namespace {
using v4f = float __attribute__((ext_vector_type(4)));

template <int LPR>
__device__ __forceinline__ float group_sum(float v) {
#pragma unroll
    for (int o = LPR / 2; o > 0; o >>= 1) v += __shfl_xor(v, o, WAVE);
    return v;
}

template <typename OT>
__device__ __forceinline__ void store4(OT* p, v4f v) {
    if constexpr (std::is_same<OT, float>::value) {
        *reinterpret_cast<v4f*>(p) = v;
    } else {
        typedef OT o4 __attribute__((ext_vector_type(4)));
        *reinterpret_cast<o4*>(p) = o4{(OT)v.x, (OT)v.y, (OT)v.z, (OT)v.w};
    }
}

template <int LPR, int NV, typename OT>
__global__ __launch_bounds__(256) void layernorm_kernel(const float* __restrict__ x, const float* __restrict__ w,
                                                       const float* __restrict__ b, OT* __restrict__ y, long rows, int cols,
                                                       float eps, unsigned* ovf) {
    float rgmax = 0.f;
    constexpr int RPW = 64 / LPR;
    const int lane = threadIdx.x & 63, sub = lane % LPR, rsel = lane / LPR;
    const long wave0 = (long)blockIdx.x * 4 + (threadIdx.x >> 6), nwaves = (long)gridDim.x * 4;
    const int n4 = cols >> 2;
    const float inv = 1.0f / (float)cols;
    for (long r0 = wave0 * RPW; r0 < rows; r0 += nwaves * RPW) {
        const long row = r0 + rsel;
        const bool rok = row < rows;
        const v4f* xr = reinterpret_cast<const v4f*>(x + (rok ? row : 0) * cols);
        v4f v[NV];
        float s = 0.f;
#pragma unroll
        for (int j = 0; j < NV; ++j) {
            const int i = sub + LPR * j;
            v[j] = (rok && i < n4) ? xr[i] : v4f{0.f, 0.f, 0.f, 0.f};
            s += (v[j].x + v[j].y) + (v[j].z + v[j].w);
        }
        const float mean = group_sum<LPR>(s) * inv;
        float q = 0.f;
#pragma unroll
        for (int j = 0; j < NV; ++j) {
            const int i = sub + LPR * j;
            if (i < n4) {
                const v4f d = v[j] - mean;
                q += (d.x * d.x + d.y * d.y) + (d.z * d.z + d.w * d.w);
            }
        }
        const float rstd = 1.0f / sqrtf(group_sum<LPR>(q) * inv + eps);
        if (!rok) continue;
        OT* yr = y + row * cols;
#pragma unroll
        for (int j = 0; j < NV; ++j) {
            const int i = sub + LPR * j;
            if (i < n4) {
                const v4f ww = reinterpret_cast<const v4f*>(w)[i], bb = reinterpret_cast<const v4f*>(b)[i];
                const v4f o = (v[j] - mean) * rstd * ww + bb;
                if constexpr (std::is_same<OT, _Float16>::value) rgmax = rg_absmax4(rgmax, o);
                store4<OT>(yr + 4 * i, o);
            }
        }
    }
    if constexpr (std::is_same<OT, _Float16>::value) rg_report(rgmax, ovf, 2u);
}

template <typename OT>
__global__ __launch_bounds__(256) void layernorm_generic_kernel(const float* __restrict__ x, const float* __restrict__ w,
                                                               const float* __restrict__ b, OT* __restrict__ y, long rows,
                                                               int cols, float eps, unsigned* ovf) {
    float rgmax = 0.f;
    const int lane = threadIdx.x & 63;
    const long wave0 = (long)blockIdx.x * 4 + (threadIdx.x >> 6), nwaves = (long)gridDim.x * 4;
    for (long row = wave0; row < rows; row += nwaves) {
        const float* xr = x + row * cols;
        float s = 0.f;
        for (int i = lane; i < cols; i += 64) s += xr[i];
        const float mean = wave_sum(s) / (float)cols;
        float q = 0.f;
        for (int i = lane; i < cols; i += 64) { const float d = xr[i] - mean; q += d * d; }
        const float rstd = 1.0f / sqrtf(wave_sum(q) / (float)cols + eps);
        for (int i = lane; i < cols; i += 64) {
            const float o = (xr[i] - mean) * rstd * w[i] + b[i];
            if constexpr (std::is_same<OT, _Float16>::value) rgmax = rg_absmax1(rgmax, o);
            y[row * cols + i] = (OT)o;
        }
    }
    if constexpr (std::is_same<OT, _Float16>::value) rg_report(rgmax, ovf, 2u);
}

template <typename OT>
int launch_ln(const float* x, const float* weight, const float* bias, OT* y, int rows, int cols, float eps, hipStream_t st) {
    unsigned* ovf = std::is_same<OT, _Float16>::value ? mi355::range_word(st) : nullptr;
    MI355_TRACE(st, "layernorm_kernel<%s> rows=%d cols=%d", std::is_same<OT, float>::value ? "out32" : "out16", rows, cols);
    const bool vec = (cols % 4 == 0) && aligned16(x) && aligned16(y) && aligned16(weight) && aligned16(bias);
#define LN(LPR_, NV_)                                                                                                \
    do {                                                                                                             \
        const long waves = ((long)rows + (64 / LPR_) - 1) / (64 / LPR_);                                            \
        const int grid = (int)((waves + 3) / 4 < 8192 ? (waves + 3) / 4 : 8192);                                    \
        layernorm_kernel<LPR_, NV_, OT><<<grid, 256, 0, st>>>(x, weight, bias, y, rows, cols, eps, ovf);                \
    } while (0)
    if (vec && cols <= 64)        LN(16, 1);
    else if (vec && cols <= 128)  LN(32, 1);
    else if (vec && cols <= 256)  LN(64, 1);
    else if (vec && cols <= 512)  LN(64, 2);
    else if (vec && cols <= 1024) LN(64, 4);
    else if (vec && cols <= 2048) LN(64, 8);
    else {
        const int grid = cdiv(rows, 4) < 8192 ? cdiv(rows, 4) : 8192;
        layernorm_generic_kernel<OT><<<grid, 256, 0, st>>>(x, weight, bias, y, rows, cols, eps, ovf);
    }
#undef LN
    return MI355_OK;
}
}

extern "C" {

int mi355_layernorm_fwd(const float* x, const float* weight, const float* bias, float* y, int rows, int cols, float eps,
                        mi355_stream_t stream) {
    MI355_CHECK_ARG(x && weight && bias && y && rows > 0 && cols > 0);
    launch_ln<float>(x, weight, bias, y, rows, cols, eps, static_cast<hipStream_t>(stream));
    MI355_LAUNCH_CHECK();
    return MI355_OK;
}

int mi355_layernorm16_fwd(const float* x, const float* weight, const float* bias, void* y16, int rows, int cols, float eps,
                          int precision, mi355_stream_t stream) {
    MI355_CHECK_ARG(x && weight && bias && y16 && rows > 0 && cols > 0);
    MI355_CHECK_ARG(precision == MI355_PREC_FP16 || precision == MI355_PREC_BF16);
    hipStream_t st = static_cast<hipStream_t>(stream);
    if (precision == MI355_PREC_FP16) launch_ln<_Float16>(x, weight, bias, static_cast<_Float16*>(y16), rows, cols, eps, st);
    else                              launch_ln<__bf16>(x, weight, bias, static_cast<__bf16*>(y16), rows, cols, eps, st);
    MI355_LAUNCH_CHECK();
    return MI355_OK;
}

}

namespace {
typedef unsigned int u4 __attribute__((ext_vector_type(4)));
template <typename T, int KC>
__global__ __launch_bounds__(256) void layernorm16_t_kernel(const float* __restrict__ x, const float* __restrict__ w, const float* __restrict__ b,
                                                           T* __restrict__ ut, int N, int C, int NP, float eps) {
    extern __shared__ unsigned int lds_t[];
    const int t = threadIdx.x, lane = t & 63, wave = t >> 6;
    const int n0 = blockIdx.x * 32, img = blockIdx.y;
    float wv[KC], bv[KC];
#pragma unroll
    for (int k = 0; k < KC; ++k) {
        const int c = lane + 64 * k;
        wv[k] = c < C ? w[c] : 0.f; bv[k] = c < C ? b[c] : 0.f;
    }
    const float inv = 1.f / (float)C;
#pragma unroll 1
    for (int pr = 0; pr < 4; ++pr) {
        const int tp = wave * 4 + pr;
        const int na = n0 + 2 * tp, nb = na + 1;
        float va[KC], vb[KC];
        const float* ra = x + ((long)img * N + (na < N ? na : 0)) * C;
        const float* rb = x + ((long)img * N + (nb < N ? nb : 0)) * C;
        float sa = 0.f, sb = 0.f;
#pragma unroll
        for (int k = 0; k < KC; ++k) {
            const int c = lane + 64 * k;
            va[k] = c < C ? ra[c] : 0.f; vb[k] = c < C ? rb[c] : 0.f;
            sa += va[k]; sb += vb[k];
        }
        sa = wave_sum(sa) * inv; sb = wave_sum(sb) * inv;
        float qa = 0.f, qb = 0.f;
#pragma unroll
        for (int k = 0; k < KC; ++k) {
            const int c = lane + 64 * k;
            const float da = c < C ? va[k] - sa : 0.f, db = c < C ? vb[k] - sb : 0.f;
            qa += da * da; qb += db * db;
        }
        const float ia = rsqrtf(wave_sum(qa) * inv + eps), ib = rsqrtf(wave_sum(qb) * inv + eps);
#pragma unroll
        for (int k = 0; k < KC; ++k) {
            const int c = lane + 64 * k;
            if (c >= C) continue;
            const T ha = na < N ? (T)((va[k] - sa) * ia * wv[k] + bv[k]) : (T)0.f;
            const T hb = nb < N ? (T)((vb[k] - sb) * ib * wv[k] + bv[k]) : (T)0.f;
            lds_t[c * 17 + tp] = (unsigned int)__builtin_bit_cast(unsigned short, ha) | ((unsigned int)__builtin_bit_cast(unsigned short, hb) << 16);
        }
    }
    __syncthreads();
    for (int idx = t; idx < C * 4; idx += 256) {
        const int c = idx >> 2, q = idx & 3;
        const unsigned int* p = lds_t + c * 17 + q * 4;
        u4 o{p[0], p[1], p[2], p[3]};
        *reinterpret_cast<u4*>(ut + ((long)img * C + c) * NP + n0 + q * 8) = o;
    }
}
}

extern "C" int mi355_layernorm16_t_fwd(const float* x, const float* weight, const float* bias, void* ut16, int B, int N, int C, int NP,
                                       float eps, int precision, mi355_stream_t stream) {
    MI355_CHECK_ARG(x && weight && bias && ut16 && B > 0 && N > 0 && C > 0 && NP >= N);
    MI355_CHECK_ARG(precision == MI355_PREC_FP16 || precision == MI355_PREC_BF16);
    if ((NP & 31) || C > 1024 || !aligned16(ut16))
        return mi355::fail(MI355_EUNSUPPORTED, "mi355_layernorm16_t_fwd: needs NP %% 32 == 0 and C <= 1024 (NP=%d C=%d)", NP, C);
    hipStream_t st = static_cast<hipStream_t>(stream);
    const dim3 grid(NP / 32, B);
    const size_t lds = (size_t)C * 17 * 4;
    MI355_TRACE(st, "layernorm16_t_kernel B=%d N=%d C=%d NP=%d", B, N, C, NP);
#define LNT(T_, KC_) layernorm16_t_kernel<T_, KC_><<<grid, 256, lds, st>>>(x, weight, bias, static_cast<T_*>(ut16), N, C, NP, eps)
#define LNT_BY_C(T_) do { if (C <= 256) LNT(T_, 4); else if (C <= 512) LNT(T_, 8); else LNT(T_, 16); } while (0)
    if (precision == MI355_PREC_FP16) LNT_BY_C(_Float16); else LNT_BY_C(__bf16);
#undef LNT_BY_C
#undef LNT
    MI355_LAUNCH_CHECK();
    return MI355_OK;
}

namespace {
__global__ __launch_bounds__(256) void token_mean_kernel(const float* __restrict__ x, float* __restrict__ y, int N, int C, long batch_stride,
                                                        int slabs) {
    const int b = blockIdx.x / slabs, c = (blockIdx.x % slabs) * 256 + threadIdx.x;
    if (c >= C) return;
    const float* p = x + (long)b * batch_stride + c;
    float s0 = 0.f, s1 = 0.f, s2 = 0.f, s3 = 0.f;
    int n = 0;
    for (; n + 3 < N; n += 4) {
        s0 += p[(long)n * C]; s1 += p[(long)(n + 1) * C]; s2 += p[(long)(n + 2) * C]; s3 += p[(long)(n + 3) * C];
    }
    for (; n < N; ++n) s0 += p[(long)n * C];
    y[(long)b * C + c] = ((s0 + s1) + (s2 + s3)) / (float)N;
}
}

extern "C" int mi355_token_mean_fwd(const float* x, float* y, int B, int N, int C, long batch_stride, mi355_stream_t stream) {
    MI355_CHECK_ARG(x && y && B > 0 && N > 0 && C > 0 && batch_stride >= (long)N * C);
    const int slabs = cdiv(C, 256);
    token_mean_kernel<<<B * slabs, 256, 0, static_cast<hipStream_t>(stream)>>>(x, y, N, C, batch_stride, slabs);
    MI355_LAUNCH_CHECK();
    return MI355_OK;
}
```

### pytorch-attention_amd/mi355attn/_ffi.py

```python
import collections
import ctypes
import os
import threading
import warnings

import torch

_HERE = os.path.dirname(os.path.abspath(__file__))
LIB_PATH = os.path.join(_HERE, "lib", "libmi355attn.so")
ABI_VERSION = 1

_lib = None
_lock = threading.Lock()

c_f32p = ctypes.c_void_p
c_int = ctypes.c_int
c_size = ctypes.c_size_t
c_vp = ctypes.c_void_p
c_float = ctypes.c_float

SIGNATURES = {
    "mi355_version": (c_int, []),
    "mi355_last_error": (ctypes.c_char_p, []),
    "mi355_set_option": (c_int, [ctypes.c_char_p, ctypes.c_long]),
    "mi355_set_default_option": (c_int, [ctypes.c_char_p, ctypes.c_long]),
    "mi355_get_option": (ctypes.c_long, [ctypes.c_char_p]),
    "mi355_workspace_forget": (c_int, [c_vp, ctypes.c_size_t]),
    "mi355_trace_begin": (c_int, []),
    "mi355_trace_end": (ctypes.c_long, [ctypes.c_char_p, c_size]),
    "mi355_sync_status": (c_int, []),
    "mi355_range_status": (c_int, []),
    "mi355_range_arm": (c_int, [c_int]),
    "mi355_range_wait": (c_int, []),
    "mi355_range_launches": (ctypes.c_long, []),
    "mi355_se_workspace_bytes": (c_size, [c_int] * 4),
    "mi355_se_fwd": (c_int, [c_vp, c_vp, c_vp, c_vp] + [c_int] * 5 + [c_vp, c_size, c_vp]),
    "mi355_se_ex_fwd": (c_int, [c_vp] * 6 + [c_int] * 6 + [c_vp, ctypes.c_size_t, c_vp]),
    "mi355_eca_workspace_bytes": (c_size, [c_int] * 4),
    "mi355_eca_fwd": (c_int, [c_vp, c_vp, c_vp] + [c_int] * 5 + [c_vp, c_size, c_vp]),
    "mi355_cbam_workspace_bytes": (c_size, [c_int] * 4),
    "mi355_cbam_fwd": (c_int, [c_vp] * 5 + [c_int] * 7 + [c_vp, c_size, c_vp]),
    "mi355_se16_fwd": (c_int, [c_vp, c_vp, c_vp, c_vp] + [c_int] * 6 + [c_vp, c_size, c_vp]),
    "mi355_eca16_fwd": (c_int, [c_vp, c_vp, c_vp] + [c_int] * 6 + [c_vp, c_size, c_vp]),
    "mi355_cbam16_workspace_bytes": (c_size, [c_int] * 4),
    "mi355_cbam16_fwd": (c_int, [c_vp] * 5 + [c_int] * 8 + [c_vp, c_size, c_vp]),
    "mi355_double_attn_workspace_bytes": (c_size, [c_int] * 6),
    "mi355_double_attn_ws_bytes": (c_size, [c_int] * 7),
    "mi355_double_attn_fwd": (c_int, [c_vp] * 10 + [c_int] * 7 + [c_vp, c_size, c_vp]),
    "mi355_linear_fwd": (c_int, [c_vp] * 6 + [c_int] * 7 + [c_vp]),
    "mi355_token_mix_fwd": (c_int, [c_vp] * 5 + [c_int] * 6 + [c_vp]),
    "mi355_layernorm_fwd": (c_int, [c_vp] * 4 + [c_int, c_int, c_float, c_vp]),
    "mi355_sdpa_fwd": (c_int, [c_vp, c_vp, c_int, c_int, c_int, c_int, c_float, c_int, c_vp]),
    "mi355_cswin_lepe_attn_fwd": (c_int, [c_vp] * 4 + [c_int] * 8 + [c_float, c_int, c_vp]),
    "mi355_xca_fwd": (c_int, [c_vp, c_vp, c_vp] + [c_int] * 5 + [c_vp]),
    "mi355_xca16_fwd": (c_int, [c_vp, c_int, c_vp, c_vp] + [c_int] * 5 + [c_vp]),
    "mi355_lpi_workspace_bytes": (c_size, [c_int] * 4),
    "mi355_lpi_fwd": (c_int, [c_vp] * 7 + [c_float] + [c_vp] * 5 + [c_int] * 4 + [c_vp, c_size, c_vp]),
    "mi355_ln_lpi_fwd": (c_int, [c_vp] * 3 + [c_float] + [c_vp] * 6 + [c_float] + [c_vp] * 5 + [c_int] * 4 + [c_vp, c_size, c_vp]),
    "mi355_patch_embed_fwd": (c_int, [c_vp] * 6 + [c_int] * 7 + [c_vp]),
    "mi355_patch_embed_workspace_bytes": (c_size, [c_int] * 7),
    "mi355_patch_embed_ws_fwd": (c_int, [c_vp] * 6 + [c_int] * 7 + [c_vp, c_size, c_vp]),
    "mi355_cast16_fwd": (c_int, [c_vp, c_vp, c_size, c_int, c_vp]),
    "mi355_layernorm16_fwd": (c_int, [c_vp] * 4 + [c_int, c_int, c_float, c_int, c_vp]),
    "mi355_ln_linear16_fwd": (c_int, [c_vp] * 4 + [c_int] * 5 + [c_float, c_int, c_int, c_int, c_vp]),
    "mi355_layernorm16_t_fwd": (c_int, [c_vp] * 4 + [c_int] * 4 + [c_float, c_int, c_vp]),
    "mi355_mixer_token_workspace_bytes": (c_size, [c_int] * 3),
    "mi355_mixer_token_fwd": (c_int, [c_vp] * 3 + [c_float] + [c_vp] * 5 + [c_int] * 5 + [c_vp, c_size, c_vp]),
    "mi355_linear16_tr_fwd": (c_int, [c_vp] * 5 + [c_int] * 6 + [c_vp]),
    "mi355_linear16_fwd": (c_int, [c_vp] * 6 + [c_int] * 8 + [c_vp]),
    "mi355_linear16_workspace_bytes": (c_size, [c_int] * 3),
    "mi355_linear16_ws_fwd": (c_int, [c_vp] * 6 + [c_int] * 8 + [c_vp, c_size, c_vp]),
    "mi355_sdpa16_fwd": (c_int, [c_vp, c_vp, c_int, c_int, c_int, c_int, c_float, c_int, c_vp]),
    "mi355_cswin_lepe_attn16_fwd": (c_int, [c_vp] * 4 + [c_int] * 8 + [c_float, c_int, c_vp]),
    "mi355_qkv_split16_fwd": (c_int, [c_vp] * 6 + [c_int] * 4 + [c_vp]),
    "mi355_sdpa16_split_fwd": (c_int, [c_vp, c_vp, c_int, c_int, c_int, c_int, c_float, c_vp]),
    "mi355_conv2d_tokens_fwd": (c_int, [c_vp] * 5 + [c_int] * 13 + [c_vp]),
    "mi355_token_mean_fwd": (c_int, [c_vp, c_vp, c_int, c_int, c_int, ctypes.c_long, c_vp]),
    "mi355_chan_stat_workspace_bytes": (ctypes.c_size_t, [c_int, c_int]),
    "mi355_simam_fwd": (c_int, [c_vp, c_vp] + [c_int] * 4 + [ctypes.c_float, c_vp, ctypes.c_size_t, c_vp]),
    "mi355_srm_fwd": (c_int, [c_vp] * 6 + [ctypes.c_float, c_vp] + [c_int] * 4 + [c_vp, ctypes.c_size_t, c_vp]),
    "mi355_gct_gauss_fwd": (c_int, [c_vp, c_vp] + [c_int] * 4 + [ctypes.c_float, ctypes.c_float, c_vp, ctypes.c_size_t, c_vp]),
    "mi355_lct_fwd": (c_int, [c_vp] * 4 + [c_int] * 5 + [ctypes.c_float, c_vp, ctypes.c_size_t, c_vp]),
    "mi355_gct_fwd": (c_int, [c_vp] * 5 + [c_int] * 4 + [ctypes.c_float, c_int, c_int, c_vp, ctypes.c_size_t, c_vp]),
    "mi355_axis_attn_workspace_bytes": (ctypes.c_size_t, [c_int] * 4),
    "mi355_gc_fwd": (c_int, [c_vp] * 10 + [c_int] * 5 + [ctypes.c_float, c_vp, ctypes.c_size_t, c_vp]),
    "mi355_coordatt_fwd": (c_int, [c_vp] * 10 + [c_int] * 5 + [c_vp, ctypes.c_size_t, c_vp]),
    "mi355_triplet_fwd": (c_int, [c_vp] * 6 + [c_int] * 5 + [c_vp, ctypes.c_size_t, c_vp]),
    "mi355_bam_workspace_bytes": (ctypes.c_size_t, [c_int] * 5),
    "mi355_bam_fwd": (c_int, [c_vp] * 3 + [c_int] * 6 + [c_vp, ctypes.c_size_t, c_vp]),
    "mi355_bam_gates_fwd": (c_int, [c_vp] * 4 + [c_int] * 6 + [c_vp, ctypes.c_size_t, c_vp]),
    "mi355_zpool_fwd": (c_int, [c_vp, c_vp] + [c_int] * 4 + [c_vp]),
    "mi355_attention_gate_workspace_bytes": (ctypes.c_size_t, [c_int] * 3),
    "mi355_attention_gate_fwd": (c_int, [c_vp] * 4 + [c_int] * 5 + [c_vp, ctypes.c_size_t, c_vp]),
    "mi355_ln_fold_stats_bytes": (ctypes.c_size_t, [c_int] * 2),
    "mi355_ln_center16_fwd": (c_int, [c_vp] * 4 + [c_int, c_int, c_float, c_int, c_vp]),
    "mi355_ln_finalize_fwd": (c_int, [c_vp] * 5 + [c_int, c_int, c_float, c_float, c_int, c_vp, c_vp]),
    "mi355_linear16_emit_fwd": (c_int, [c_vp] * 5 + [c_int] * 6 + [c_vp] * 4),
    "mi355_linear16_lnfold_fwd": (c_int, [c_vp] * 6 + [c_int] * 7 + [c_vp]),
    "mi355_mhsa_workspace_bytes": (ctypes.c_size_t, [c_int] * 4),
    "mi355_mhsa_fwd": (c_int, [c_vp, c_int] + [c_vp] * 6 + [c_int] * 4 + [c_float, c_int, c_vp, ctypes.c_size_t, c_vp]),
    "mi355_sk_workspace_bytes": (ctypes.c_size_t, [c_int] * 4),
    "mi355_sk_fwd": (c_int, [c_vp] * 3 + [c_int] * 7 + [c_vp, ctypes.c_size_t, c_vp]),
    "mi355_cam_workspace_bytes": (ctypes.c_size_t, [c_int] * 2),
    "mi355_cam_fwd": (c_int, [c_vp] * 3 + [c_int] * 5 + [c_vp, ctypes.c_size_t, c_vp]),
    "mi355_tokens_to_nchw_axpy_fwd": (c_int, [c_vp] * 4 + [c_int] * 3 + [c_vp]),
    "mi355_dwconv_nchw_tokens_fwd": (c_int, [c_vp] * 4 + [c_int] * 5 + [c_vp]),
    "mi355_qk_logits_fwd": (c_int, [c_vp] * 3 + [c_int] * 8 + [c_vp]),
    "mi355_topk_mask_fwd": (c_int, [c_vp, ctypes.c_long, c_int, c_int, c_vp]),
    "mi355_adaptive_pool_tokens_fwd": (c_int, [c_vp] * 2 + [c_int] * 6 + [c_vp]),
    "mi355_dwconv3x3_tokens_residual_fwd": (c_int, [c_vp] * 4 + [c_int] * 4 + [ctypes.c_long, c_vp]),
    "mi355_mlp_fused_fwd": (c_int, [c_vp] * 7 + [ctypes.c_long, c_int, c_int, c_int, ctypes.c_float, c_int, c_vp]),
    "mi355_proj_mlp_fused_fwd": (c_int, [c_vp] * 10 + [ctypes.c_long, c_int, c_int, c_int, ctypes.c_float, c_int, c_vp]),
    "mi355_sdpa_general_fwd": (c_int, [c_vp] * 5 + [c_int] * 5 + [ctypes.c_long] * 5 + [ctypes.c_float, c_int, c_int, c_vp]),
    "mi355_dwconv_patch_tokens_fwd": (c_int, [c_vp] * 4 + [c_int] * 5 + [c_vp]),
    "mi355_cswin_lepe_attn16_pair_fwd": (c_int, [c_vp] * 6 + [c_int] * 5 + [ctypes.c_float, c_int, c_vp]),
    "mi355_cswin_stripe_attn_fwd": (c_int, [c_vp] * 8 + [c_int] * 5 + [c_float, c_float, c_int, c_vp]),
    "mi355_class_attn_fwd": (c_int, [c_vp] * 4 + [c_int] * 4 + [ctypes.c_long, ctypes.c_long, ctypes.c_float, c_vp]),
    "mi355_axpby_fwd": (c_int, [c_vp] * 4 + [ctypes.c_long, c_int, ctypes.c_long, ctypes.c_long, ctypes.c_long, ctypes.c_float, c_vp]),
    "mi355_comm_unique_id": (c_int, [c_vp, c_size]),
    "mi355_comm_init": (c_int, [c_vp, c_size, c_int, c_int, ctypes.POINTER(c_vp)]),
    "mi355_allgather_f32": (c_int, [c_vp, c_vp, c_vp, c_size, c_vp]),
    "mi355_comm_destroy": (c_int, [c_vp]),
    "mi355_bicubic_rows_fwd": (c_int, [c_vp, c_vp] + [c_int] * 5 + [c_float, c_float, c_vp]),
    "mi355_stream_copy": (c_int, [c_vp, c_vp, c_size, c_vp]),
    "mi355_stream_read": (c_int, [c_vp, c_size, c_vp, c_vp]),
    "mi355_mfma_yardstick": (c_int, [c_int, c_int, c_vp, c_vp, c_vp]),
    "mi355_event_time_begin": (c_int, [c_vp, ctypes.POINTER(c_vp)]),
    "mi355_event_time_end": (c_int, [c_vp, c_vp, ctypes.POINTER(c_float)]),
    "mi355_linear16_x32_fwd": (c_int, [c_vp] * 4 + [c_int] * 7 + [c_vp]),
    "mi355_linear16_stats_fwd": (c_int, [c_vp] * 5 + [c_int] * 6 + [c_vp, c_float, c_vp]),
    "mi355_linear16_ln16_fwd": (c_int, [c_vp] * 7 + [c_float, c_vp] + [c_int] * 7 + [c_vp]),
    "mi355_ln_lpi_stats_fwd": (c_int, [c_vp] * 10 + [c_float] + [c_vp] * 5 + [c_int] * 4 + [c_vp]),
    "mi355_sdpa_core_fwd": (c_int, [c_vp, c_vp, c_int, c_int, c_int, c_int, c_float, c_int, c_vp]),
    "mi355_sdpa_core_workspace_bytes": (c_size, [c_int] * 4),
    "mi355_gemm_bias_act_fwd": (c_int, [c_vp] * 6 + [c_int] * 7 + [c_vp]),
    "mi355_gemm_bias_act_workspace_bytes": (c_size, [c_int] * 3),
    "mi355_mixer_token_mlp_fwd": (c_int, [c_vp] * 3 + [c_float] + [c_vp] * 5 + [c_int] * 5 + [c_vp, c_size, c_vp]),
    "mi355_mixer_token_mlp_workspace_bytes": (c_size, [c_int] * 3),
    "mi355_cswin_lepe_attn_workspace_bytes": (c_size, [c_int] * 3),
    "mi355_xca_workspace_bytes": (c_size, [c_int] * 4),
    "mi355_layernorm_workspace_bytes": (c_size, [c_int] * 2),
}


class Mi355Error(RuntimeError):
    pass


class Mi355RangeError(Mi355Error):
    """A finite value saturated to inf in an fp16 operand tensor of an earlier launch (include/mi355attn.h mi355_range_status)."""


def lib():
    global _lib
    if _lib is not None:
        return _lib
    with _lock:
        if _lib is not None:
            return _lib
        if not os.path.exists(LIB_PATH):
            raise Mi355Error(
                f"{LIB_PATH} is missing: build it with `python pytorch-attention_amd/build.py` "
                "(hipcc --offload-arch=gfx950).  There is no CPU/eager fallback for the MI355X path.")
        handle = ctypes.CDLL(LIB_PATH)
        for name, (res, args) in SIGNATURES.items():
            fn = getattr(handle, name)
            fn.restype = res
            fn.argtypes = args
        v = handle.mi355_version()
        if v != ABI_VERSION:
            raise Mi355Error(f"libmi355attn ABI version {v} != binding version {ABI_VERSION}; rebuild")
        handle.mi355_set_default_option(b"ws_persistent", 1)
        _lib = handle
    return _lib


MI355_EUNSUPPORTED = -2
MI355_ERANGE = -5


def check(code, what):
    if code != 0:
        msg = lib().mi355_last_error()
        raise Mi355Error(f"{what} failed (code {code}): {msg.decode() if msg else '?'}")


def stream_ptr(device=None):
    if device is not None and device.type == "cuda" and device.index is not None and device.index != torch.cuda.current_device():
        raise Mi355Error(f"tensor on {device} but the current device is cuda:{torch.cuda.current_device()}: "
                         "wrap the call in `with torch.cuda.device(x.device):` (kernels launch on the current device)")
    return ctypes.c_void_p(torch.cuda.current_stream(device).cuda_stream)


def dptr(t):
    return ctypes.c_void_p(t.data_ptr()) if t is not None else ctypes.c_void_p(0)


def require_device_f32(t, name):
    if not isinstance(t, torch.Tensor):
        raise TypeError(f"{name}: expected a torch.Tensor, got {type(t).__name__}")
    if not t.is_cuda:
        raise Mi355Error(
            f"{name} lives on {t.device}: the mi355attn modules only run on an MI355X device tensor "
            "(move the module and its input to 'cuda'); there is no CPU path in this package.")
    if t.dtype != torch.float32:
        raise TypeError(f"{name}: expected float32, got {t.dtype} (16-bit activations are accepted by SELayer, ECALayer, CBAM, "
                        "ChannelAttention and SpatialAttention only)")
    if t.requires_grad and torch.is_grad_enabled():
        _warn_no_autograd()
    return t if t.is_contiguous() else t.contiguous()


IO_CODES = {torch.float16: 1, torch.bfloat16: 2}


def require_device_io(t, name):
    if isinstance(t, torch.Tensor) and t.is_cuda and t.dtype in IO_CODES:
        if t.requires_grad and torch.is_grad_enabled():
            _warn_no_autograd()
        return (t if t.is_contiguous() else t.contiguous()), IO_CODES[t.dtype]
    if isinstance(t, torch.Tensor) and not t.is_cuda and t.dtype in IO_CODES:
        t = t.new_empty(0, dtype=torch.float32)
    return require_device_f32(t, name), 0


_warned_autograd = False


def _warn_no_autograd():
    global _warned_autograd
    if not _warned_autograd:
        _warned_autograd = True
        warnings.warn("mi355attn is a forward-only engine: a tensor that requires grad entered a kernel with autograd enabled; "
                      "the output has no grad_fn and no gradient will flow through this module (use torch.no_grad() / "
                      "requires_grad_(False) to silence this)", RuntimeWarning, stacklevel=4)


_ws_cache = {}


def _capturing():
    return torch.cuda.is_current_stream_capturing()


def workspace(nbytes, device):
    if _capturing():
        return torch.empty(max(int(nbytes), 256), dtype=torch.uint8, device=device)
    key = (device.index if device.index is not None else torch.cuda.current_device(),
           torch.cuda.current_stream(device).cuda_stream)
    t = _ws_cache.get(key)
    if t is None or t.numel() < nbytes:
        t = torch.empty(max(int(nbytes), 1 << 20), dtype=torch.uint8, device=device)
        _ws_cache[key] = t
# ... 84 lines not shown
```

### pytorch-attention_amd/mi355attn/functional.py

```python
import ctypes
import threading
import weakref

import torch

from . import _ffi
from ._ffi import check, dptr, lib, require_device_f32, stream_ptr, workspace

PREC_STRICT, PREC_FP16, PREC_BF16 = 0, 1, 2
PREC_LOGIT = 3
ACT_NONE, ACT_GELU, ACT_RELU = 0, 1, 2

_default_precision = PREC_FP16


class _StrictOverride(threading.local):
    depth = 0


_strict_override = _StrictOverride()
_strict_active = 0
_strict_lock = threading.Lock()


# ... 901 lines not shown
    check(lib().mi355_mixer_token_fwd(dptr(x), dptr(require_device_f32(norm.weight, "norm.weight")), dptr(require_device_f32(norm.bias, "norm.bias")),
                                      float(norm.eps), dptr(w1p), dptr(require_device_f32(fc1.bias, "fc1.bias")), dptr(w2s),
                                      dptr(require_device_f32(fc2.bias, "fc2.bias")), dptr(y), B, N, C, T, p, dptr(ws), ws.numel(),
                                      stream_ptr(x.device)), "mi355_mixer_token_fwd")
    return y


def linear16_tr(xt16, w16, bias, resid, precision=None):
    xt16 = _require16(xt16, "xt16", precision)
    w16 = _require16(w16, "w16", precision)
    bias, resid = _opt(bias, "bias"), _opt(resid, "resid")
    B, C, K = xt16.shape
    N = w16.shape[0]
    if w16.shape[1] != K:
        raise ValueError(f"linear16_tr: weight in_features {w16.shape[1]} != {K}")
    if resid is not None and tuple(resid.shape) != (B, N, C):
        raise ValueError("linear16_tr: residual shape mismatch")
    y = torch.empty(B, N, C, dtype=torch.float32, device=xt16.device)
    check(lib().mi355_linear16_tr_fwd(dptr(xt16), dptr(w16), dptr(bias), dptr(resid), dptr(y), B * C, N, K, K, C, _prec(precision),
                                      stream_ptr(xt16.device)), "mi355_linear16_tr_fwd")
    return y


def weight16_padk(w, K, precision=None):
    def build():
        out = torch.zeros(w.shape[0], K, dtype=dtype16(precision), device=w.device)
        out[:, :w.shape[1]] = w.detach()
        return out
    tag = (w._version, w.data_ptr(), tuple(w.shape))
    return _derived_get((w,), ("w16padk", K, _prec(precision)), tag, build)


LN_FOLD_TOL = 1.0


class LnState:
    __slots__ = ("a16", "rowtau", "cvec")

    def __init__(self, a16, rowtau, cvec):
        self.a16, self.rowtau, self.cvec = a16, rowtau, cvec


def ln_fold_enabled():
    return _ffi.get_option("ln_fold") == 1


def ln_fold_ok(rows, C, N, K, precision=None):
    return (_prec(precision) in (PREC_FP16, PREC_BF16) and rows % 128 == 0 and N == C and C % 256 == 0 and C <= 2048 and
            K % 64 == 0 and K >= 640 and _ffi.get_option("ln_fold") == 1 and rows * C * 4 < (1 << 31))


def lnfold_weights(ln, lin, precision=None):
    p = _prec(precision)
    anchors = (ln.weight, ln.bias, lin.weight) + ((lin.bias,) if lin.bias is not None else ())
    tag = tuple((t._version, t.data_ptr()) for t in anchors)

    def build():
        w = lin.weight.detach()
        wg = w * ln.weight.detach()[None, :]
        if p == PREC_FP16 and not bool((wg.abs() < 65504.0).all()):
            return None
        w16 = wg.to(dtype16(p)).contiguous()
        colsum = w16.double().sum(dim=1).float().contiguous()
        b = w.double() @ ln.bias.detach().double()
        if lin.bias is not None:
            b = b + lin.bias.detach().double()
        return w16, colsum, b.float().contiguous()

    return _derived_get(anchors, ("lnfold", p), tag, build)


def ln_center16(x, eps=1e-5, precision=None):
    p = _prec(precision)
    x = require_device_f32(x, "x")
    C = x.shape[-1]
    rows = x.numel() // C
    a16 = torch.empty(x.shape, dtype=dtype16(p), device=x.device)
    rowtau = torch.empty(rows, 2, dtype=torch.float32, device=x.device)
    cvec = torch.empty(rows, dtype=torch.float32, device=x.device)
    check(lib().mi355_ln_center16_fwd(dptr(x), dptr(a16), dptr(rowtau), dptr(cvec), rows, C, float(eps), p, stream_ptr(x.device)),
          "mi355_ln_center16_fwd")
    return LnState(a16, rowtau, cvec)


def linear16_lnfold(state, w16, bias, colsum, act=ACT_NONE, precision=None):
    _range_check()
    p = _prec(precision)
    a16 = _require16(state.a16, "a16", p)
    w16 = _require16(w16, "w16", p)
    N, K = w16.shape
    if a16.shape[-1] != K:
        raise ValueError(f"linear16_lnfold: operand width {a16.shape[-1]} != weight in_features {K}")
    M = a16.numel() // K
    y = torch.empty(*a16.shape[:-1], N, dtype=dtype16(p), device=a16.device)
    check(lib().mi355_linear16_lnfold_fwd(dptr(a16), dptr(w16), dptr(_opt(bias, "bias")), dptr(state.rowtau), dptr(colsum), dptr(y),
                                          M, N, K, K, N, act, p, stream_ptr(a16.device)), "mi355_linear16_lnfold_fwd")
    return y


def linear16_emit(x16, w16, bias, resid, cvec, eps=1e-5, act=ACT_NONE, precision=None, slow_rows=None):
    _range_check()
    p = _prec(precision)
    x16 = _require16(x16, "x16", p)
    w16 = _require16(w16, "w16", p)
    N, K = w16.shape
    if x16.shape[-1] != K:
        raise ValueError(f"linear16_emit: x last dim {x16.shape[-1]} != weight in_features {K}")
    M = x16.numel() // K
    resid = _opt(resid, "resid")
    if resid is not None and resid.numel() != M * N:
        raise ValueError("linear16_emit: residual shape mismatch")
    dev = x16.device
    y = torch.empty(*x16.shape[:-1], N, dtype=torch.float32, device=dev)
    a16 = torch.empty(*x16.shape[:-1], N, dtype=dtype16(p), device=dev)
    stats = _ffi.workspace_named("ln_fold_stats", lib().mi355_ln_fold_stats_bytes(M, N), dev)
    rowtau = torch.empty(M, 2, dtype=torch.float32, device=dev)
    check(lib().mi355_linear16_emit_fwd(dptr(x16), dptr(w16), dptr(_opt(bias, "bias")), dptr(resid), dptr(y), M, N, K, K, act, p,
                                        dptr(cvec), dptr(a16), dptr(stats), stream_ptr(dev)), "mi355_linear16_emit_fwd")
    check(lib().mi355_ln_finalize_fwd(dptr(stats), dptr(y), dptr(a16), dptr(cvec), dptr(rowtau), M, N, float(eps), float(LN_FOLD_TOL), p,
                                      dptr(slow_rows), stream_ptr(dev)), "mi355_ln_finalize_fwd")
    return y, LnState(a16, rowtau, cvec)


def mhsa16(x, wqkv16, bqkv, wproj16, bproj, num_heads, scale, resid=None, precision=None):
    _range_check()
    p = _prec(precision)
    x_is16 = x.dtype != torch.float32
    x = _require16(x, "x", p) if x_is16 else require_device_f32(x, "x")
    wqkv16, wproj16 = _require16(wqkv16, "wqkv16", p), _require16(wproj16, "wproj16", p)
    B, N, C = x.shape
    if tuple(wqkv16.shape) != (3 * C, C) or tuple(wproj16.shape) != (C, C):
        raise ValueError("mhsa16: weight shapes do not match the embedding width")
    bqkv, bproj, resid = _opt(bqkv, "qkv.bias"), _opt(bproj, "proj.bias"), _opt(resid, "resid")
    if resid is not None and resid.numel() != x.numel():
        raise ValueError("mhsa16: residual shape mismatch")
    y = torch.empty(B, N, C, dtype=torch.float32, device=x.device)
    nws = lib().mi355_mhsa_workspace_bytes(B, N, C, 1 if x_is16 else 0)
    ws = _ffi.workspace_named("mhsa", nws, x.device)
    check(lib().mi355_mhsa_fwd(dptr(x), 1 if x_is16 else 0, dptr(wqkv16), dptr(bqkv), dptr(wproj16), dptr(bproj), dptr(resid), dptr(y),
                               B, N, C, int(num_heads), float(scale), p, dptr(ws), nws, stream_ptr(x.device)), "mi355_mhsa_fwd")
    return y


def sdpa16(qkv16, num_heads, scale, precision=None):
    qkv16 = _require16(qkv16, "qkv16", precision)
    B, N, C3 = qkv16.shape
    C = C3 // 3
    out = torch.empty(B, N, C, dtype=qkv16.dtype, device=qkv16.device)
    check(lib().mi355_sdpa16_fwd(dptr(qkv16), dptr(out), B, N, num_heads, C // num_heads, float(scale), _prec(precision),
                                 stream_ptr(qkv16.device)), "mi355_sdpa16_fwd")
    return out


def logit_envelope(C, K, num_heads, n_tokens):
    return C % num_heads == 0 and C // num_heads in (32, 64) and n_tokens <= 224 and K % 64 == 0 and C % 64 == 0


def qkv_split16(x, w_hi, w_lo, w_v16, bias=None):
    _range_check()
    x = require_device_f32(x, "x")
    C2, K = w_hi.shape
    C = C2 // 2
    if x.shape[-1] != K or tuple(w_lo.shape) != (C2, K) or tuple(w_v16.shape) != (C, K):
        raise ValueError("qkv_split16: weight parts do not match each other or x")
    for t_, name, dt in ((w_hi, "w_hi", torch.bfloat16), (w_lo, "w_lo", torch.bfloat16), (w_v16, "w_v16", torch.float16)):
        if not t_.is_cuda or t_.dtype != dt or not t_.is_contiguous():
            raise TypeError(f"qkv_split16: {name} must be a contiguous {dt} device tensor")
    bias = _opt(bias, "bias")
    M = x.numel() // K
    y = torch.empty(*x.shape[:-1], 5 * C, dtype=torch.int16, device=x.device)
    check(lib().mi355_qkv_split16_fwd(dptr(x), dptr(w_hi), dptr(w_lo), dptr(w_v16), dptr(bias), dptr(y), M, C, K, K,
                                      stream_ptr(x.device)), "mi355_qkv_split16_fwd")
    return y


def qkv_split16_planes(qkv5):
    C = qkv5.shape[-1] // 5
    planes = [qkv5[..., i * C:(i + 1) * C] for i in range(5)]
    return tuple(p_.view(torch.bfloat16) for p_ in planes[:4]) + (planes[4].view(torch.float16),)


def sdpa16_split(qkv5, num_heads, scale):
    if not qkv5.is_cuda or qkv5.dtype != torch.int16 or qkv5.dim() != 3:
        raise TypeError("sdpa16_split: expected the (B, N, 5C) int16 device tensor qkv_split16 returns")
    qkv5 = qkv5 if qkv5.is_contiguous() else qkv5.contiguous()
    B, N, C5 = qkv5.shape
    C = C5 // 5
    out = torch.empty(B, N, C, dtype=torch.float16, device=qkv5.device)
    check(lib().mi355_sdpa16_split_fwd(dptr(qkv5), dptr(out), B, N, int(num_heads), C // num_heads, float(scale),
                                       stream_ptr(qkv5.device)), "mi355_sdpa16_split_fwd")
    return out


def cswin_lepe_attention16(qkv16, getv_w, getv_b, out16, reso, c0, Cb, heads, Hsp, Wsp, scale, precision=None):
    qkv16 = _require16(qkv16, "qkv16", precision)
    getv_w = require_device_f32(getv_w, "get_v.weight")
    getv_b = require_device_f32(getv_b, "get_v.bias")
    B = qkv16.shape[0]
    Ctot = qkv16.shape[-1] // 3
    check(lib().mi355_cswin_lepe_attn16_fwd(dptr(qkv16), dptr(getv_w), dptr(getv_b), dptr(out16), B, reso, Ctot, c0, Cb, heads,
                                            Hsp, Wsp, float(scale), _prec(precision), stream_ptr(qkv16.device)),
          "mi355_cswin_lepe_attn16_fwd")
    return out16


def sdpa(qkv, num_heads, scale, precision=None):
    qkv = require_device_f32(qkv, "qkv")
    B, N, C3 = qkv.shape
    C = C3 // 3
    d = C // num_heads
    out = torch.empty(B, N, C, dtype=torch.float32, device=qkv.device)
    check(lib().mi355_sdpa_fwd(dptr(qkv), dptr(out), B, N, num_heads, d, float(scale), _prec(precision),
                               stream_ptr(qkv.device)), "mi355_sdpa_fwd")
    return out


def cswin_lepe_attention(qkv, getv_w, getv_b, out, reso, c0, Cb, heads, Hsp, Wsp, scale, precision=None):
    qkv = require_device_f32(qkv, "qkv")
    getv_w = require_device_f32(getv_w, "get_v.weight")
    getv_b = require_device_f32(getv_b, "get_v.bias")
    B, L = qkv.shape[0], qkv.shape[1]
    Ctot = qkv.shape[-1] // 3 if qkv.dim() == 3 else qkv.shape[-1]
    check(lib().mi355_cswin_lepe_attn_fwd(dptr(qkv), dptr(getv_w), dptr(getv_b), dptr(out), B, reso, Ctot, c0, Cb,
                                          heads, Hsp, Wsp, float(scale), _prec(precision), stream_ptr(qkv.device)),
          "mi355_cswin_lepe_attn_fwd")
    return out


def xca_core(qkv, temperature, num_heads, precision=None, out16=False):
    temperature = require_device_f32(temperature, "temperature").reshape(-1)
    B, N, C3 = qkv.shape
    C = C3 // 3
    if out16:
        is16 = qkv.dtype == dtype16(precision)
        if not is16:
            qkv = require_device_f32(qkv, "qkv")
        elif not (qkv.is_cuda and qkv.is_contiguous()):
            raise ValueError("xca_core: 16-bit qkv must be a contiguous device tensor")
        out = torch.empty(B, N, C, dtype=dtype16(precision), device=qkv.device)
        check(lib().mi355_xca16_fwd(dptr(qkv), 1 if is16 else 0, dptr(temperature), dptr(out), B, N, num_heads, C // num_heads,
                                    _prec(precision), stream_ptr(qkv.device)), "mi355_xca16_fwd")
        return out
    qkv = require_device_f32(qkv, "qkv")
    out = torch.empty(B, N, C, dtype=torch.float32, device=qkv.device)
    check(lib().mi355_xca_fwd(dptr(qkv), dptr(temperature), dptr(out), B, N, num_heads, C // num_heads,
                              _prec(precision), stream_ptr(qkv.device)), "mi355_xca_fwd")
    return out


def lpi(x, w1, b1, bn_w, bn_b, bn_mean, bn_var, bn_eps, w2, b2, H, W, gamma=None, resid=None, ln=None, stats=None):
    x = require_device_f32(x, "x")
    B, N, C = x.shape
    if N != H * W:
        raise ValueError(f"lpi: {N} tokens do not form a {H}x{W} grid")
    pre = [require_device_f32(t, n) for t, n in ((w1, "conv1.weight"), (b1, "conv1.bias"), (bn_w, "bn.weight"),
                                                 (bn_b, "bn.bias"), (bn_mean, "bn.running_mean"),
                                                 (bn_var, "bn.running_var"))]
    post = [require_device_f32(t, n) for t, n in ((w2, "conv2.weight"), (b2, "conv2.bias"))]
    gamma, resid = _opt(gamma, "gamma"), _opt(resid, "resid")
    y = torch.empty_like(x)
    n = lib().mi355_lpi_workspace_bytes(B, H, W, C)
    ws = workspace(n, x.device)
    if ln is not None and stats is not None:
        lw, lb = require_device_f32(ln.weight, "ln.weight"), require_device_f32(ln.bias, "ln.bias")
        stats = require_device_f32(stats, "stats")
        if stats.numel() != B * N * 2:
            raise ValueError("lpi: stats must hold (mean, rstd) for every token")
        check(lib().mi355_ln_lpi_stats_fwd(dptr(x), dptr(stats), dptr(lw), dptr(lb), *[dptr(a) for a in pre], float(bn_eps),
                                           *[dptr(a) for a in post], dptr(gamma), dptr(resid), dptr(y), B, H, W, C, stream_ptr(x.device)),
              "mi355_ln_lpi_stats_fwd")
        return y
    if ln is not None:
        lw, lb = require_device_f32(ln.weight, "ln.weight"), require_device_f32(ln.bias, "ln.bias")
        check(lib().mi355_ln_lpi_fwd(dptr(x), dptr(lw), dptr(lb), float(ln.eps), *[dptr(a) for a in pre], float(bn_eps),
                                     *[dptr(a) for a in post], dptr(gamma), dptr(resid), dptr(y), B, H, W, C, dptr(ws), ws.numel(),
                                     stream_ptr(x.device)), "mi355_ln_lpi_fwd")
        return y
    check(lib().mi355_lpi_fwd(dptr(x), *[dptr(a) for a in pre], float(bn_eps), *[dptr(a) for a in post], dptr(gamma),
                              dptr(resid), dptr(y), B, H, W, C, dptr(ws), ws.numel(), stream_ptr(x.device)),
          "mi355_lpi_fwd")
    return y


def patch_embed(img, wp, bp, cls, pos, patch, precision=None):
    img = require_device_f32(img, "img")
    wp = require_device_f32(wp, "proj.weight")
    E = wp.shape[0]
    wp = wp.reshape(E, -1)
    bp = require_device_f32(bp, "proj.bias")
    cls, pos = _opt(cls, "cls_token"), _opt(pos, "pos")
    B, Cin, H, W = img.shape
    P = (H // patch) * (W // patch)
    if (cls is None) != (pos is None):
        raise ValueError("patch_embed: pass both cls and pos (ViT) or neither (plain patches)")
    if pos is not None and pos.numel() != (P + 1) * E:
        raise ValueError("patch_embed: position embedding does not match the patch grid")
    tokens = torch.empty(B, P + (1 if cls is not None else 0), E, dtype=torch.float32, device=img.device)
    n = lib().mi355_patch_embed_workspace_bytes(B, Cin, H, W, patch, E, _prec(precision)) if cls is not None else 0
    if n:
        ws = _ffi.workspace_named("patch_embed", n, img.device)
        check(lib().mi355_patch_embed_ws_fwd(dptr(img), dptr(wp), dptr(bp), dptr(cls), dptr(pos), dptr(tokens), B, Cin, H, W,
                                             patch, E, _prec(precision), dptr(ws), ws.numel(), stream_ptr(img.device)),
              "mi355_patch_embed_ws_fwd")
        return tokens
    check(lib().mi355_patch_embed_fwd(dptr(img), dptr(wp), dptr(bp), dptr(cls), dptr(pos), dptr(tokens), B, Cin, H, W,
                                      patch, E, _prec(precision), stream_ptr(img.device)), "mi355_patch_embed_fwd")
# ... 306 lines not shown
```

### pytorch-attention_amd/mi355attn/modules/vit.py

```python
import torch
from torch import nn

from .. import functional as F


def _bias(lin):
    return lin.bias if lin.bias is not None else None


def _fast(precision, *linears):
    return F._prec(precision) != F.PREC_STRICT and all(F.fast_gemm_ok(l.in_features, l.out_features) for l in linears)


def _mlp16(x, fc1, fc2, precision, second_gelu, gamma=None, resid=None):
    p = F._prec(precision)
    h16 = F.cast_linear16(x, F.weight16(fc1.weight, p), fc1.bias, act=F.ACT_GELU, precision=p)
    folded = F.weight16_scaled(fc2.weight, fc2.bias, gamma, p) if gamma is not None and not second_gelu else None
    if folded is not None:
        w16, b = folded
        return F.linear16(h16, w16, b, resid=resid, precision=p)
    return F.linear16(h16, F.weight16(fc2.weight, p), fc2.bias, act=F.ACT_GELU if second_gelu else F.ACT_NONE, gamma=gamma,
                      resid=resid, precision=p)


# ... 16 lines not shown
    def __init__(self, dim, num_heads=4, qkv_bias=False, attn_drop=0, proj_drop=0, precision=None):
        super().__init__()
        assert dim % num_heads == 0
        self.num_heads = num_heads
        self.scale = (dim // num_heads) ** -0.5
        self.qkv = nn.Linear(dim, dim * 3, bias=qkv_bias)
        self.proj = nn.Linear(dim, dim)
        self.precision = precision
        self.attn_drop, self.proj_drop = attn_drop, proj_drop

    def fast_ok(self, n_tokens=None):
        d = self.qkv.in_features // self.num_heads
        return _fast(self.precision, self.qkv, self.proj) and d in F.SDPA_WIDTHS

    def _core(self, qkv, fast):
        B, N, C3 = qkv.shape
        C = C3 // 3
        d = C // self.num_heads
        if d in (32, 64) and N <= 224:
            return F.sdpa16(qkv, self.num_heads, self.scale, precision=self.precision) if fast else \
                F.sdpa(qkv, self.num_heads, self.scale, precision=self.precision)
        return F.sdpa_general(qkv[..., :C], qkv[..., C:2 * C], qkv[..., 2 * C:], self.num_heads, self.scale, precision=self.precision)

    def _forward_logit(self, x, resid):
        C = self.qkv.in_features
        if not F.logit_envelope(C, C, self.num_heads, x.shape[-2]):
            with F._forced_strict(self):
                return self.forward(x, resid)
        x = x if x.dtype == torch.float32 else x.float()
        qkv5 = F.qkv_split16(x, *F.weight_split16(self.qkv.weight), _bias(self.qkv))
        ctx = F.sdpa16_split(qkv5, self.num_heads, self.scale)
        return F.linear16(ctx, F.weight16(self.proj.weight, F.PREC_FP16), self.proj.bias, resid=resid, precision=F.PREC_FP16)

    def forward(self, x, resid=None):
        if F.logit_mode(self.precision):
            return self._forward_logit(x, resid)
        d = self.qkv.in_features // self.num_heads
        if d not in F.SDPA_WIDTHS:
            from .mhsa import _fused_qkv_attention
            out, _, _ = _fused_qkv_attention(x if x.dtype == torch.float32 else x.float(), self.qkv, self.proj, self.num_heads, d,
                                             self.scale, self.precision)
            return out if resid is None else F.axpby(out, torch.empty_like(out), out.numel() // out.shape[-1], out.shape[-1],
                                                     out.shape[-1], out.shape[-1], u=resid, ldu=out.shape[-1])
        if self.fast_ok():
            p = F._prec(self.precision)
            return F.mhsa16(x, F.weight16(self.qkv.weight, p), _bias(self.qkv), F.weight16(self.proj.weight, p), self.proj.bias,
                            self.num_heads, self.scale, resid=resid, precision=p)
        qkv = F.linear(x, self.qkv.weight, _bias(self.qkv), precision=self.precision)
        ctx = self._core(qkv, False)
        return F.linear(ctx, self.proj.weight, self.proj.bias, resid=resid, precision=self.precision)


class PatchEmbedding(nn.Module):
    def __init__(self, image_size=224, patch_size=16, in_channels=3, embedding_dim=768):
        super().__init__()
        assert image_size % patch_size == 0
        self.patch_size = patch_size
        self.num_patches = (image_size // patch_size) ** 2
        self.proj = nn.Conv2d(in_channels, embedding_dim, kernel_size=patch_size, stride=patch_size)
        self.precision = None

    def forward(self, x):
        return F.patch_embed(x, self.proj.weight, self.proj.bias, None, None, self.patch_size, self.precision)


class TransformerEncoder(nn.Module):
    def __init__(self, dim, num_heads=4, mlp_ratio=4, qkv_bias=False, attn_drop=0, proj_drop=0, precision=None):
        super().__init__()
        self.attn = Attention(dim, num_heads, qkv_bias, attn_drop, proj_drop, precision)
        self.layernorm1 = nn.LayerNorm(dim)
        self.mlp = Mlp(dim, int(dim * mlp_ratio))
        self.mlp.precision = precision
        self.layernorm2 = nn.LayerNorm(dim)

    def _norm(self, ln, x, fast):
        if fast:
            return F.layernorm16(x, ln.weight, ln.bias, ln.eps, F._prec(self.attn.precision))
        return F.layernorm(x, ln.weight, ln.bias, ln.eps)

    def forward(self, x):
        if self.fold_ok(x):
            return self.forward_folded(x)[0]
        return self.forward_plain(x)

    def forward_plain(self, x):
        if F.logit_mode(self.attn.precision):
            x = self.attn(F.layernorm(x, self.layernorm1.weight, self.layernorm1.bias, self.layernorm1.eps), resid=x)
            return self.mlp(self._norm(self.layernorm2, x, _fast(self.attn.precision, self.mlp.fc1, self.mlp.fc2)), resid=x)
        fast = self.attn.fast_ok(x.shape[1]) and _fast(self.attn.precision, self.mlp.fc1, self.mlp.fc2)
        x = self.attn(self._norm(self.layernorm1, x, fast), resid=x)
        return self.mlp(self._norm(self.layernorm2, x, fast), resid=x)

    def fold_ok(self, x):
        if not F.ln_fold_enabled() or x.dim() != 3 or x.dtype != torch.float32 or not x.is_cuda:
            return False
        if F.logit_mode(self.attn.precision):
            return False
        B, N, C = x.shape
        p = F._prec(self.attn.precision)
        d = C // self.attn.num_heads
        if not (self.attn.fast_ok(N) and _fast(p, self.mlp.fc1, self.mlp.fc2) and d in (32, 64) and N <= 224):
            return False
        if not (F.ln_fold_ok(B * N, C, C, C, p) and F.ln_fold_ok(B * N, C, C, self.mlp.fc1.out_features, p)):
            return False
        return (F.lnfold_weights(self.layernorm1, self.attn.qkv, p) is not None and
                F.lnfold_weights(self.layernorm2, self.mlp.fc1, p) is not None)

    def forward_folded(self, x, state=None, next_eps=None):
        p = F._prec(self.attn.precision)
        ln1, ln2, at, mlp = self.layernorm1, self.layernorm2, self.attn, self.mlp
        wq, sq, bq = F.lnfold_weights(ln1, at.qkv, p)
        w1, s1, b1 = F.lnfold_weights(ln2, mlp.fc1, p)
        if state is None:
            state = F.ln_center16(x, ln1.eps, p)
        qkv = F.linear16_lnfold(state, wq, bq, sq, precision=p)
        ctx = F.sdpa16(qkv, at.num_heads, at.scale, precision=p)
        x1, st = F.linear16_emit(ctx, F.weight16(at.proj.weight, p), at.proj.bias, x, state.cvec, ln2.eps, precision=p)
        h = F.linear16_lnfold(st, w1, b1, s1, act=F.ACT_GELU, precision=p)
        w2 = F.weight16(mlp.fc2.weight, p)
        if next_eps is None:
            return F.linear16(h, w2, mlp.fc2.bias, act=F.ACT_GELU, resid=x1, precision=p), None
        return F.linear16_emit(h, w2, mlp.fc2.bias, x1, st.cvec, next_eps, act=F.ACT_GELU, precision=p)


class VisionTransformer(nn.Module):
    def __init__(self, image_size=224, patch_size=16, in_channels=3, depths=12, num_heads=4, mlp_ratio=4,
                 embedding_dim=768, qkv_bias=False, attn_drop=0, proj_drop=0, global_pool="token",
                 num_classes=1000, precision=None):
        super().__init__()
        self.patch_embedding = PatchEmbedding(image_size, patch_size, in_channels, embedding_dim)
        self.patch_embedding.precision = precision
        self.global_pool = global_pool
        self.precision = precision
        n = self.patch_embedding.num_patches
        self.cls_token = nn.Parameter(torch.zeros(1, 1, embedding_dim))
        self.position_embedding = nn.Parameter(torch.zeros(1, n + 1, embedding_dim))
        self.blocks = nn.Sequential(*(TransformerEncoder(embedding_dim, num_heads, mlp_ratio, qkv_bias, attn_drop,
                                                         proj_drop, precision) for _ in range(depths)))
        self.head = nn.Linear(embedding_dim, num_classes)
        nn.init.trunc_normal_(self.position_embedding, std=.02)
        nn.init.trunc_normal_(self.cls_token, std=.02)
        self.apply(self._reset)

    @staticmethod
    def _reset(m):
        if isinstance(m, nn.Linear):
            nn.init.trunc_normal_(m.weight, std=.02)
            if m.bias is not None:
                nn.init.zeros_(m.bias)
        elif isinstance(m, nn.LayerNorm):
            nn.init.zeros_(m.bias)
            nn.init.ones_(m.weight)

    def forward(self, x):
        B, _, H, W = x.shape
        ps = self.patch_embedding.patch_size
        pos = F.vit_pos_table(self.position_embedding, ps, H, W)
        tok = F.patch_embed(x, self.patch_embedding.proj.weight, self.patch_embedding.proj.bias,
                            self.cls_token.reshape(-1), pos, ps, self.precision)
        blocks, state = list(self.blocks), None
        elig = [blk.fold_ok(tok) for blk in blocks] if F.ln_fold_enabled() else None
        for i, blk in enumerate(blocks):
            if elig is not None and elig[i]:
                nxt_ok = i + 1 < len(blocks) and elig[i + 1]
                tok, state = blk.forward_folded(tok, state, blocks[i + 1].layernorm1.eps if nxt_ok else None)
            else:
                tok, state = blk(tok), None
        if self.global_pool == "token":
            pooled = tok[:, 0]
        elif self.global_pool == "avg":
            pooled = F.token_mean(tok, skip_first=1)
        else:
            pooled = tok
        return F.linear(pooled, self.head.weight, self.head.bias, precision=self.precision)
```

Before: 16130 images/s.

## Compute only the class-token row in the final ViT block when pooling by token

With token pooling, only the class-token row of the last encoder block reaches the head, so a dedicated tail path handles that block differently. It runs LayerNorm 1 on all tokens, computes K and V for every token, and computes Q for row 0 only. A query-limited variant of the attention kernel then attends for that single row, and the projection, LayerNorm 2 and MLP run on just B rows through a small 32x64 GEMM tile. This removes most of the projection and MLP work in the last block, at the cost of extra launches, a new attention template instantiation and a narrower eligibility check (it is disabled when LN folding or forward hooks are active).

```diff
diff --git a/include/mi355attn.h b/include/mi355attn.h
--- a/include/mi355attn.h
+++ b/include/mi355attn.h
@@ -264,6 +264,15 @@
                    const float* resid, float* y, int B, int N, int C, int heads, float scale, int precision, void* workspace,
                    size_t workspace_bytes, mi355_stream_t stream);
 
+int mi355_sdpa16_rows_fwd(const void* qkv16, void* out16, int B, int N, int heads, int d, float scale, int q_rows, int out_rows,
+                          int precision, mi355_stream_t stream);
+
+size_t mi355_vit_tail_workspace_bytes(int B, int N, int C, int hidden);
+int mi355_vit_tail_fwd(const float* x, const float* ln1_w, const float* ln1_b, float eps1, const void* Wqkv16, const float* b_qkv,
+                       const void* Wproj16, const float* b_proj, const float* ln2_w, const float* ln2_b, float eps2, const void* Wfc1_16,
+                       const float* b_fc1, const void* Wfc2_16, const float* b_fc2, float* y, int B, int N, int C, int hidden, int heads,
+                       float scale, int precision, void* workspace, size_t workspace_bytes, mi355_stream_t stream);
+
 int mi355_sdpa_general_fwd(const void* q, const void* k, const void* v, const float* bias, void* out, int B, int num_heads, int Nq,
                            int Nkv, int head_dim, long ldq, long ldk, long ldv, long ldo, long bias_batch_stride, float scale,
                            int io16, int precision, mi355_stream_t stream);
diff --git a/pytorch-attention_amd/csrc/api.hip b/pytorch-attention_amd/csrc/api.hip
--- a/pytorch-attention_amd/csrc/api.hip
+++ b/pytorch-attention_amd/csrc/api.hip
@@ -13,7 +13,7 @@
 
 constexpr int MAX_DEV = 64;
 enum Opt { O_CHUNK_IMAGES, O_NT, O_REVERSE, O_GEMM_VARIANT, O_ECA_SINGLE, O_SE_SINGLE, O_CBAM_SINGLE, O_WS_PERSISTENT, O_STEM_DIRECT,
-           O_ZOO_SINGLE, O_SPIN_LIMIT, O_GEMM_PA, O_GEMM_SPLITK, O_DA_FUSED, O_DA_RANGES, O_SE_OCC, O_LN_FOLD, O_GEMM_PA16, O_GEMM_PA_BLOCK, O_GEMM_PA_TAIL, O_LPI_PATCH, O_MIXER_FUSED, O_MIXER_EARLY, O_GEMM_SMALL, O_MLP_TT4, O_MIXER_STATS, O_ATTN_NW, O_GEMM_W4, O_RANGE_FALLBACK, O_GEMM_WREG, O_XCA_TR, O_MLP_WIDE, O_GEMM_WST, O_GEMM_WSLAB, O_IO16_OCC, O_COUNT };
+           O_ZOO_SINGLE, O_SPIN_LIMIT, O_GEMM_PA, O_GEMM_SPLITK, O_DA_FUSED, O_DA_RANGES, O_SE_OCC, O_LN_FOLD, O_GEMM_PA16, O_GEMM_PA_BLOCK, O_GEMM_PA_TAIL, O_LPI_PATCH, O_MIXER_FUSED, O_MIXER_EARLY, O_GEMM_SMALL, O_MLP_TT4, O_MIXER_STATS, O_ATTN_NW, O_GEMM_W4, O_RANGE_FALLBACK, O_GEMM_WREG, O_XCA_TR, O_MLP_WIDE, O_GEMM_WST, O_GEMM_WSLAB, O_IO16_OCC, O_VIT_TAIL, O_COUNT };
 struct OptDesc { const char* key; long def, lo, hi; };
 static const OptDesc kOpts[O_COUNT] = {
     {"chunk_images", 0, 0, 1L << 40},
@@ -51,6 +51,7 @@
     {"gemm_wst", 0, 0, 4},
     {"gemm_wslab", 1, 0, 2},
     {"io16_occ", 4, 2, 4},
+    {"vit_tail", 1, 0, 1},
 };
 static_assert(sizeof(kOpts) / sizeof(kOpts[0]) == O_COUNT, "one table row per option, in enum order");
 namespace {
@@ -111,6 +112,7 @@
 long opt_mlp_wide() { return opt(O_MLP_WIDE); }
 long opt_gemm_wst() { return opt(O_GEMM_WST); }
 long opt_gemm_wslab() { return opt(O_GEMM_WSLAB); }
+long opt_vit_tail() { return opt(O_VIT_TAIL); }
 
 namespace {
 struct WsEntry { unsigned long long key; };
diff --git a/pytorch-attention_amd/csrc/attn.hip b/pytorch-attention_amd/csrc/attn.hip
--- a/pytorch-attention_amd/csrc/attn.hip
+++ b/pytorch-attention_amd/csrc/attn.hip
@@ -26,16 +26,21 @@
 struct AttnPairRg : AttnPair {
     unsigned* ovf;
 };
-template <bool IO16>
-using attn_kargs = typename std::conditional<IO16, AttnPair, AttnPairRg>::type;
+struct AttnPairQ : AttnPair {
+    int q_tiles, q_rows;
+    int out_rows;
+};
+template <bool IO16, bool QLIM = false>
+using attn_kargs = typename std::conditional<QLIM, AttnPairQ, typename std::conditional<IO16, AttnPair, AttnPairRg>::type>::type;
 template <bool IO16>
 const attn_kargs<IO16>& attn_pick(const AttnPairRg& p) { return p; }
 
 #ifndef MI355_ATTN_FMA_SM
 #define MI355_ATTN_FMA_SM 1
 #endif
-template <int PREC, int D, int KT, bool LEPE, bool IO16, int NW, int OCC = 1, int TFULL = -1>
-__global__ __launch_bounds__(NW * 64, OCC) void win_attn_kernel(const attn_kargs<IO16> pr) {
+template <int PREC, int D, int KT, bool LEPE, bool IO16, int NW, int OCC = 1, int TFULL = -1, bool QLIM = false>
+__global__ __launch_bounds__(NW * 64, OCC) void win_attn_kernel(const attn_kargs<IO16, QLIM> pr) {
+    static_assert(!QLIM || (IO16 && !LEPE), "the query limit exists for the plain 16-bit-I/O core");
     constexpr bool FMA_SM = MI355_ATTN_FMA_SM != 0;
     const int lid = xcd_contiguous_block();
     const bool second = lid >= pr.split;
@@ -75,7 +80,14 @@
     auto tok = [&](int s) { const int r = srow(s); return (wy0 + r) * a.reso + wx0 + (s - r * a.Wsp); };
 
     const int l15 = lane & 15, g = lane >> 4;
-    const int nqt = (T + 15) >> 4;
+    int nqt = (T + 15) >> 4;
+    int qmax = T;
+    if constexpr (QLIM) {
+        nqt = pr.q_tiles < nqt ? pr.q_tiles : nqt;
+        qmax = pr.q_rows < T ? pr.q_rows : T;
+    }
+    int orows = a.L;
+    if constexpr (QLIM) orows = pr.out_rows;
     constexpr int NQ = (KT + NW - 1) / NW;
     const rsrc_t img_rs = make_rsrc(IO16 ? static_cast<const void*>(base) : nullptr, IO16 ? (bufops_u32)((long)a.L * row3 * sizeof(gel)) : 0u);
     auto ld16 = [&](bool live, int token, int el_off) -> v8 {
@@ -88,8 +100,9 @@
         for (int iq = 0; iq < NQ; ++iq) {
             const int qs = (wave + iq * NW) * 16 + l15;
             const int tq = tok(qs < T ? qs : 0);
-#pragma unroll
-            for (int ks = 0; ks < D / 32; ++ks) qraw[iq][ks] = ld16(qs < T, tq, ks * 32 + g * 8);
+            const bool ql = QLIM ? (qs < qmax && wave + iq * NW < nqt) : qs < T;
+#pragma unroll
+            for (int ks = 0; ks < D / 32; ++ks) qraw[iq][ks] = ld16(ql, tq, ks * 32 + g * 8);
         }
     }
     __shared__ float s_lw[LEPE ? D * 10 : 1];
@@ -352,8 +365,8 @@
             for (int it = 0; it < 16 / RPI; ++it) {
                 const int r = it * RPI + lane / LPR, c8 = (lane % LPR) * 8;
                 const int qslot = qt * 16 + r;
-                if (qslot < T)
-                    *reinterpret_cast<v8*>(static_cast<gel*>(a.out) + ((long)b * a.L + tok(qslot)) * a.Ctot + och0 + c8) =
+                if (QLIM ? qslot < qmax : qslot < T)
+                    *reinterpret_cast<v8*>(static_cast<gel*>(a.out) + ((long)b * orows + tok(qslot)) * a.Ctot + och0 + c8) =
                         *reinterpret_cast<const v8*>(slab + r * OP + c8);
             }
         } else {
@@ -416,15 +429,38 @@
     return MI355_OK;
 }
 
-}
-
-static int sdpa_common(const void* qkv, void* out, int B, int N, int heads, int d, float scale, int precision, bool io16,
-                       hipStream_t st) {
+template <int D>
+int launch_attn_rows(const AttnArgs& a, int B, int q_rows, int out_rows, int precision, hipStream_t st) {
+    AttnPairQ pr{};
+    pr.a0 = a;
+    pr.split = B * a.nwin * a.heads;
+    pr.q_rows = q_rows;
+    pr.q_tiles = (q_rows + 15) >> 4;
+    pr.out_rows = out_rows;
+    const int grid = pr.split;
+    MI355_TRACE(st, "win_attn_kernel<d=%d,io16,rows> B=%d heads=%d tokens=%d q_rows=%d", D, B, a.heads, a.T, q_rows);
+#define GOQ(P, KT_, NW_) win_attn_kernel<P, D, KT_, false, true, NW_, 1, -1, true><<<grid, NW_ * 64, 0, st>>>(pr)
+#define BYKTQ(P) do { if (a.T <= 64) GOQ(P, 4, 4); else if (a.T <= 128) GOQ(P, 8, 4); else GOQ(P, 14, 8); } while (0)
+    if (precision == MI355_PREC_FP16) BYKTQ(1); else BYKTQ(2);
+#undef BYKTQ
+#undef GOQ
+    return MI355_OK;
+}
+
+}
+
+static AttnArgs sdpa_args(const void* qkv, void* out, int N, int heads, int d, float scale) {
     AttnArgs a{};
     a.qkv = qkv; a.out = out; a.L = N; a.Ctot = heads * d; a.c0 = 0; a.heads = heads;
     a.koff = a.Ctot; a.voff = 2 * a.Ctot; a.oc0 = 0;
     a.reso = N; a.Hsp = 1; a.Wsp = N; a.nWx = 1; a.nwin = 1; a.T = N; a.scale = scale; a.pre_scale = 0;
     a.wsp_magic = (unsigned)(((1ull << 32) + (unsigned)N - 1) / (unsigned)N);
+    return a;
+}
+
+static int sdpa_common(const void* qkv, void* out, int B, int N, int heads, int d, float scale, int precision, bool io16,
+                       hipStream_t st) {
+    const AttnArgs a = sdpa_args(qkv, out, N, heads, d, scale);
     if (d == 64) return io16 ? launch_attn<64, false, true>(a, B, precision, st) : launch_attn<64, false, false>(a, B, precision, st);
     return io16 ? launch_attn<32, false, true>(a, B, precision, st) : launch_attn<32, false, false>(a, B, precision, st);
 }
@@ -478,6 +514,19 @@
     SDPA_CHECKS("mi355_sdpa16_fwd");
     int rc = sdpa_common(qkv, out, B, N, heads, d, scale, precision, true, static_cast<hipStream_t>(stream));
     if (rc) return rc;
+    MI355_LAUNCH_CHECK();
+    return MI355_OK;
+}
+
+int mi355_sdpa16_rows_fwd(const void* qkv, void* out, int B, int N, int heads, int d, float scale, int q_rows, int out_rows, int precision,
+                          mi355_stream_t stream) {
+    SDPA_CHECKS("mi355_sdpa16_rows_fwd");
+    MI355_CHECK_ARG(q_rows > 0 && q_rows <= N && out_rows >= q_rows);
+    MI355_CHECK_ARG(precision == MI355_PREC_FP16 || precision == MI355_PREC_BF16);
+    const AttnArgs a = sdpa_args(qkv, out, N, heads, d, scale);
+    hipStream_t st = static_cast<hipStream_t>(stream);
+    if (d == 64) launch_attn_rows<64>(a, B, q_rows, out_rows, precision, st);
+    else         launch_attn_rows<32>(a, B, q_rows, out_rows, precision, st);
     MI355_LAUNCH_CHECK();
     return MI355_OK;
 }
diff --git a/pytorch-attention_amd/csrc/common.h b/pytorch-attention_amd/csrc/common.h
--- a/pytorch-attention_amd/csrc/common.h
+++ b/pytorch-attention_amd/csrc/common.h
@@ -40,6 +40,9 @@
 long  opt_mlp_wide();
 long  opt_gemm_wst();
 long  opt_gemm_wslab();
+long  opt_vit_tail();
+int   layernorm16_rows(const float* x, long ldx, const float* add, float* xs, const float* weight, const float* bias, void* y16, int rows,
+                       int cols, float eps, int precision, hipStream_t st);
 bool  mlp_wide_applicable(int C, int hidden);
 int   mlp_wide(const float* x, const void* w1_16, const float* b1, const void* w2_16, const float* b2, const float* gamma, float* y, long M, int C,
                int layernorm, float eps, int precision, hipStream_t st);
diff --git a/pytorch-attention_amd/csrc/gemm16.h b/pytorch-attention_amd/csrc/gemm16.h
--- a/pytorch-attention_amd/csrc/gemm16.h
+++ b/pytorch-attention_amd/csrc/gemm16.h
@@ -44,5 +44,6 @@
 int gemm16_wst(const g16::G16Args& g, int out16, int precision, hipStream_t st);
 int gemm16_wslab(const g16::G16Args& g, int out16, int precision, hipStream_t st);
 int gemm16_wslab_check(const g16::G16Args& g, int precision);
+int gemm16_rows(const g16::G16Args& g, int out16, int precision, hipStream_t st);
 int linear16_dispatch(const g16::G16Args& g, int out16, int precision, void* ws, size_t ws_bytes, hipStream_t st);
 }
diff --git a/pytorch-attention_amd/csrc/gemm16.hip b/pytorch-attention_amd/csrc/gemm16.hip
--- a/pytorch-attention_amd/csrc/gemm16.hip
+++ b/pytorch-attention_amd/csrc/gemm16.hip
@@ -615,6 +615,20 @@
     return MI355_OK;
 }
 
+int mi355::gemm16_rows(const G16Args& g, int out16, int precision, hipStream_t st) {
+    const int grid = cdiv(g.M, 32) * cdiv(g.N, 64);
+    MI355_TRACE(st, "gemm16_kernel<rows 32x64,%s> M=%d N=%d K=%d%s", out16 ? "out16" : "out32", g.M, g.N, g.K, g.act == MI355_ACT_GELU ? " gelu" : "");
+    if (precision == MI355_PREC_FP16) {
+        if (out16) gemm16_kernel<_Float16, true, 32, 64, 1, 4, false, 10><<<grid, 256, 0, st>>>(g);
+        else       gemm16_kernel<_Float16, false, 32, 64, 1, 4, false, 10><<<grid, 256, 0, st>>>(g);
+    } else {
+        if (out16) gemm16_kernel<__bf16, true, 32, 64, 1, 4, false, 10><<<grid, 256, 0, st>>>(g);
+        else       gemm16_kernel<__bf16, false, 32, 64, 1, 4, false, 10><<<grid, 256, 0, st>>>(g);
+    }
+    MI355_LAUNCH_CHECK();
+    return MI355_OK;
+}
+
 extern "C" {
 
 int mi355_linear16_tr_fwd(const void* X16, const void* W16, const float* bias, const float* resid, float* Y, int M, int N, int K,
diff --git a/pytorch-attention_amd/csrc/layernorm.hip b/pytorch-attention_amd/csrc/layernorm.hip
--- a/pytorch-attention_amd/csrc/layernorm.hip
+++ b/pytorch-attention_amd/csrc/layernorm.hip
@@ -69,6 +69,78 @@
         }
     }
     if constexpr (std::is_same<OT, _Float16>::value) rg_report(rgmax, ovf, 2u);
+}
+
+template <int LPR, int NV, typename OT>
+__global__ __launch_bounds__(256) void layernorm_rows_kernel(const float* __restrict__ x, long ldx, const float* __restrict__ add,
+                                                            float* __restrict__ xs, const float* __restrict__ w, const float* __restrict__ b,
+                                                            OT* __restrict__ y, long rows, int cols, float eps, unsigned* ovf) {
+    float rgmax = 0.f;
+    constexpr int RPW = 64 / LPR;
+    const int lane = threadIdx.x & 63, sub = lane % LPR, rsel = lane / LPR;
+    const long wave0 = (long)blockIdx.x * 4 + (threadIdx.x >> 6), nwaves = (long)gridDim.x * 4;
+    const int n4 = cols >> 2;
+    const float inv = 1.0f / (float)cols;
+    for (long r0 = wave0 * RPW; r0 < rows; r0 += nwaves * RPW) {
+        const long row = r0 + rsel;
+        const bool rok = row < rows;
+        const v4f* xr = reinterpret_cast<const v4f*>(x + (rok ? row : 0) * ldx);
+        const v4f* ar = reinterpret_cast<const v4f*>(add + (rok ? row : 0) * cols);
+        v4f v[NV];
+        float s = 0.f;
+#pragma unroll
+        for (int j = 0; j < NV; ++j) {
+            const int i = sub + LPR * j;
+            v[j] = (rok && i < n4) ? xr[i] + ar[i] : v4f{0.f, 0.f, 0.f, 0.f};
+            s += (v[j].x + v[j].y) + (v[j].z + v[j].w);
+        }
+        const float mean = group_sum<LPR>(s) * inv;
+        float q = 0.f;
+#pragma unroll
+        for (int j = 0; j < NV; ++j) {
+            const int i = sub + LPR * j;
+            if (i < n4) {
+                const v4f d = v[j] - mean;
+                q += (d.x * d.x + d.y * d.y) + (d.z * d.z + d.w * d.w);
+            }
+        }
+        const float rstd = 1.0f / sqrtf(group_sum<LPR>(q) * inv + eps);
+        if (!rok) continue;
+        OT* yr = y + row * cols;
+        float* sr = xs + row * cols;
+#pragma unroll
+        for (int j = 0; j < NV; ++j) {
+            const int i = sub + LPR * j;
+            if (i < n4) {
+                const v4f ww = reinterpret_cast<const v4f*>(w)[i], bb = reinterpret_cast<const v4f*>(b)[i];
+                const v4f o = (v[j] - mean) * rstd * ww + bb;
+                if constexpr (std::is_same<OT, _Float16>::value) rgmax = rg_absmax4(rgmax, o);
+                *reinterpret_cast<v4f*>(sr + 4 * i) = v[j];
+                store4<OT>(yr + 4 * i, o);
+            }
+        }
+    }
+    if constexpr (std::is_same<OT, _Float16>::value) rg_report(rgmax, ovf, 2u);
+}
+
+template <typename OT>
+void launch_ln_rows(const float* x, long ldx, const float* add, float* xs, const float* weight, const float* bias, OT* y, int rows, int cols,
+                    float eps, hipStream_t st) {
+    unsigned* ovf = std::is_same<OT, _Float16>::value ? mi355::range_word(st) : nullptr;
+    MI355_TRACE(st, "layernorm_rows_kernel<out16> rows=%d cols=%d", rows, cols);
+#define LNR(LPR_, NV_)                                                                                                      \
+    do {                                                                                                                    \
+        const long waves = ((long)rows + (64 / LPR_) - 1) / (64 / LPR_);                                                   \
+        const int grid = (int)((waves + 3) / 4 < 8192 ? (waves + 3) / 4 : 8192);                                           \
+        layernorm_rows_kernel<LPR_, NV_, OT><<<grid, 256, 0, st>>>(x, ldx, add, xs, weight, bias, y, rows, cols, eps, ovf); \
+    } while (0)
+    if (cols <= 64)        LNR(16, 1);
+    else if (cols <= 128)  LNR(32, 1);
+    else if (cols <= 256)  LNR(64, 1);
+    else if (cols <= 512)  LNR(64, 2);
+    else if (cols <= 1024) LNR(64, 4);
+    else                   LNR(64, 8);
+#undef LNR
 }
 
 template <typename OT>
@@ -121,6 +193,17 @@
 }
 }
 
+int mi355::layernorm16_rows(const float* x, long ldx, const float* add, float* xs, const float* weight, const float* bias, void* y16, int rows,
+                            int cols, float eps, int precision, hipStream_t st) {
+    if ((cols & 3) || cols > 2048 || (ldx & 3) || !aligned16(x) || !aligned16(add) || !aligned16(xs) || !aligned16(y16) || !aligned16(weight) ||
+        !aligned16(bias))
+        return MI355_EUNSUPPORTED;
+    if (precision == MI355_PREC_FP16) launch_ln_rows<_Float16>(x, ldx, add, xs, weight, bias, static_cast<_Float16*>(y16), rows, cols, eps, st);
+    else                              launch_ln_rows<__bf16>(x, ldx, add, xs, weight, bias, static_cast<__bf16*>(y16), rows, cols, eps, st);
+    MI355_LAUNCH_CHECK();
+    return MI355_OK;
+}
+
 extern "C" {
 
 int mi355_layernorm_fwd(const float* x, const float* weight, const float* bias, float* y, int rows, int cols, float eps,
diff --git a/pytorch-attention_amd/csrc/vit_tail.hip b/pytorch-attention_amd/csrc/vit_tail.hip
--- /dev/null
+++ b/pytorch-attention_amd/csrc/vit_tail.hip
@@ -0,0 +1,92 @@
+#include "gemm16.h"
+
+using g16::G16Args;
+
+static size_t up256(size_t v) { return (v + 255) & ~(size_t)255; }
+
+namespace {
+struct TailWs {
+    size_t u16, qkv16, ctx16, t32, x1, v16, h16, lin, lin_bytes, total;
+};
+TailWs tail_ws(int B, int N, int C, int hidden) {
+    const size_t M = (size_t)B * N;
+    TailWs w{};
+    size_t o = 0;
+    w.u16 = o;   o += up256(M * C * 2);
+    w.qkv16 = o; o += up256(M * 3 * C * 2);
+    w.ctx16 = o; o += up256((size_t)B * C * 2);
+    w.t32 = o;   o += up256((size_t)B * C * 4);
+    w.x1 = o;    o += up256((size_t)B * C * 4);
+    w.v16 = o;   o += up256((size_t)B * C * 2);
+    w.h16 = o;   o += up256((size_t)B * hidden * 2);
+    w.lin = o;
+    w.lin_bytes = mi355_linear16_workspace_bytes((int)M, 2 * C, C);
+    o += up256(w.lin_bytes);
+    w.total = o + 256;
+    return w;
+}
+
+int rows_gemm(const void* X16, int ldx, const void* W16, const float* bias, const float* resid, void* Y, int ldy, int M, int N, int K, int act,
+              int out16, int precision, hipStream_t st) {
+    G16Args g{};
+    g.A = X16; g.B = W16; g.C = Y; g.bias = bias; g.resid = resid;
+    g.M = M; g.N = N; g.K = K; g.lda = ldx; g.ldb = K; g.ldc = ldy; g.act = act;
+    if (out16 && precision == MI355_PREC_FP16) g.ovf = mi355::range_word(st);
+    return mi355::gemm16_rows(g, out16, precision, st);
+}
+}
+
+extern "C" {
+
+size_t mi355_vit_tail_workspace_bytes(int B, int N, int C, int hidden) {
+    if (B <= 0 || N <= 0 || C <= 0 || hidden <= 0) return 0;
+    return tail_ws(B, N, C, hidden).total;
+}
+
+int mi355_vit_tail_fwd(const float* x, const float* ln1_w, const float* ln1_b, float eps1, const void* Wqkv16, const float* b_qkv,
+                       const void* Wproj16, const float* b_proj, const float* ln2_w, const float* ln2_b, float eps2, const void* Wfc1_16,
+                       const float* b_fc1, const void* Wfc2_16, const float* b_fc2, float* y, int B, int N, int C, int hidden, int heads,
+                       float scale, int precision, void* workspace, size_t workspace_bytes, mi355_stream_t stream) {
+    MI355_CHECK_ARG(x && ln1_w && ln1_b && Wqkv16 && Wproj16 && ln2_w && ln2_b && Wfc1_16 && Wfc2_16 && y && workspace);
+    MI355_CHECK_ARG(B > 0 && N > 0 && C > 0 && hidden > 0 && heads > 0);
+    if (!(precision == MI355_PREC_FP16 || precision == MI355_PREC_BF16))
+        return mi355::fail(MI355_EUNSUPPORTED, "mi355_vit_tail_fwd: precision 1 (fp16) or 2 (bf16) (got %d)", precision);
+    if ((C % heads) || (C % 64) || (hidden % 64) || C > 2048)
+        return mi355::fail(MI355_EUNSUPPORTED, "mi355_vit_tail_fwd: C %% heads == 0, C %% 64 == 0, C <= 2048, hidden %% 64 == 0 (C=%d heads=%d hidden=%d)",
+                           C, heads, hidden);
+    const int d = C / heads;
+    if (!(d == 32 || d == 64)) return mi355::fail(MI355_EUNSUPPORTED, "mi355_vit_tail_fwd: head_dim %d (built: 32, 64)", d);
+    if (N > 224) return mi355::fail(MI355_EUNSUPPORTED, "mi355_vit_tail_fwd: %d tokens > 224 (K/V-resident core)", N);
+    const size_t M = (size_t)B * N;
+    if (M > (size_t)0x7fffffff || (size_t)N * 3 * C > (size_t)0x7fffffff)
+        return mi355::fail(MI355_EUNSUPPORTED, "mi355_vit_tail_fwd: B * N or N * 3C too large");
+    const TailWs ws = tail_ws(B, N, C, hidden);
+    MI355_CHECK_ARG(workspace_bytes >= ws.total && aligned16(workspace));
+    MI355_CHECK_ARG(aligned16(x) && aligned16(y) && aligned16(Wqkv16) && aligned16(Wproj16) && aligned16(Wfc1_16) && aligned16(Wfc2_16));
+    MI355_CHECK_ARG(aligned16(ln1_w) && aligned16(ln1_b) && aligned16(ln2_w) && aligned16(ln2_b));
+    MI355_CHECK_ARG((!b_qkv || aligned16(b_qkv)) && (!b_proj || aligned16(b_proj)) && (!b_fc1 || aligned16(b_fc1)) && (!b_fc2 || aligned16(b_fc2)));
+    hipStream_t st = static_cast<hipStream_t>(stream);
+    char* w = static_cast<char*>(workspace);
+    void* u16 = w + ws.u16;
+    char* qkv16 = w + ws.qkv16;
+    void* ctx16 = w + ws.ctx16;
+    float* t32 = reinterpret_cast<float*>(w + ws.t32);
+    float* x1 = reinterpret_cast<float*>(w + ws.x1);
+    void* v16 = w + ws.v16;
+    void* h16 = w + ws.h16;
+    const char* Wq = static_cast<const char*>(Wqkv16);
+
+    if (int rc = mi355_layernorm16_fwd(x, ln1_w, ln1_b, u16, (int)M, C, eps1, precision, stream)) return rc;
+    if (int rc = mi355_linear16_ws_fwd(u16, Wq + (size_t)C * C * 2, b_qkv ? b_qkv + C : nullptr, nullptr, nullptr, qkv16 + (size_t)C * 2, (int)M,
+                                       2 * C, C, C, 3 * C, MI355_ACT_NONE, 1, precision, ws.lin_bytes ? w + ws.lin : nullptr, ws.lin_bytes, stream))
+        return rc;
+    if (int rc = rows_gemm(u16, N * C, Wq, b_qkv, nullptr, qkv16, N * 3 * C, B, C, C, MI355_ACT_NONE, 1, precision, st)) return rc;
+    if (int rc = mi355_sdpa16_rows_fwd(qkv16, ctx16, B, N, heads, d, scale, 1, 1, precision, stream)) return rc;
+    if (int rc = rows_gemm(ctx16, C, Wproj16, b_proj, nullptr, t32, C, B, C, C, MI355_ACT_NONE, 0, precision, st)) return rc;
+    if (int rc = mi355::layernorm16_rows(x, (long)N * C, t32, x1, ln2_w, ln2_b, v16, B, C, eps2, precision, st))
+        return rc == MI355_EUNSUPPORTED ? mi355::fail(rc, "mi355_vit_tail_fwd: LayerNorm 2 rows need C %% 4 == 0 and 16-byte aligned rows") : rc;
+    if (int rc = rows_gemm(v16, C, Wfc1_16, b_fc1, nullptr, h16, hidden, B, hidden, C, MI355_ACT_GELU, 1, precision, st)) return rc;
+    return rows_gemm(h16, hidden, Wfc2_16, b_fc2, x1, y, C, B, C, hidden, MI355_ACT_GELU, 0, precision, st);
+}
+
+}
diff --git a/pytorch-attention_amd/mi355attn/_ffi.py b/pytorch-attention_amd/mi355attn/_ffi.py
--- a/pytorch-attention_amd/mi355attn/_ffi.py
+++ b/pytorch-attention_amd/mi355attn/_ffi.py
@@ -99,6 +99,9 @@
     "mi355_linear16_lnfold_fwd": (c_int, [c_vp] * 6 + [c_int] * 7 + [c_vp]),
     "mi355_mhsa_workspace_bytes": (ctypes.c_size_t, [c_int] * 4),
     "mi355_mhsa_fwd": (c_int, [c_vp, c_int] + [c_vp] * 6 + [c_int] * 4 + [c_float, c_int, c_vp, ctypes.c_size_t, c_vp]),
+    "mi355_sdpa16_rows_fwd": (c_int, [c_vp, c_vp, c_int, c_int, c_int, c_int, c_float, c_int, c_int, c_int, c_vp]),
+    "mi355_vit_tail_workspace_bytes": (ctypes.c_size_t, [c_int] * 4),
+    "mi355_vit_tail_fwd": (c_int, [c_vp] * 3 + [c_float] + [c_vp] * 6 + [c_float] + [c_vp] * 5 + [c_int] * 5 + [c_float, c_int, c_vp, ctypes.c_size_t, c_vp]),
     "mi355_sk_workspace_bytes": (ctypes.c_size_t, [c_int] * 4),
     "mi355_sk_fwd": (c_int, [c_vp] * 3 + [c_int] * 7 + [c_vp, ctypes.c_size_t, c_vp]),
     "mi355_cam_workspace_bytes": (ctypes.c_size_t, [c_int] * 2),
diff --git a/pytorch-attention_amd/mi355attn/functional.py b/pytorch-attention_amd/mi355attn/functional.py
--- a/pytorch-attention_amd/mi355attn/functional.py
+++ b/pytorch-attention_amd/mi355attn/functional.py
@@ -1077,6 +1077,51 @@
     return out
 
 
+def sdpa16_rows(qkv16, num_heads, scale, q_rows, out=None, precision=None):
+    qkv16 = _require16(qkv16, "qkv16", precision)
+    B, N, C3 = qkv16.shape
+    C = C3 // 3
+    if out is None:
+        out = torch.empty(B, q_rows, C, dtype=qkv16.dtype, device=qkv16.device)
+    if out.dtype != qkv16.dtype or out.dim() != 3 or out.shape[0] != B or out.shape[2] != C or not out.is_contiguous():
+        raise ValueError("sdpa16_rows: out must be a dense (B, out_rows, C) tensor of qkv16's type")
+    check(lib().mi355_sdpa16_rows_fwd(dptr(qkv16), dptr(out), B, N, num_heads, C // num_heads, float(scale), int(q_rows), out.shape[1],
+                                      _prec(precision), stream_ptr(qkv16.device)), "mi355_sdpa16_rows_fwd")
+    return out
+
+
+def vit_tail_enabled():
+    return _ffi.get_option("vit_tail") == 1
+
+
+def vit_tail_envelope(C, hidden, num_heads, n_tokens):
+    return (C % num_heads == 0 and C // num_heads in (32, 64) and n_tokens <= 224 and C % 64 == 0 and C <= 2048 and hidden % 64 == 0)
+
+
+def vit_tail16(x, ln1, wqkv16, bqkv, wproj16, bproj, ln2, wfc1_16, bfc1, wfc2_16, bfc2, num_heads, scale, precision=None):
+    _range_check()
+    p = _prec(precision)
+    x = require_device_f32(x, "x")
+    B, N, C = x.shape
+    hidden = wfc1_16.shape[0]
+    ws16 = [_require16(t, n, p) for t, n in ((wqkv16, "wqkv16"), (wproj16, "wproj16"), (wfc1_16, "wfc1_16"), (wfc2_16, "wfc2_16"))]
+    if [tuple(t.shape) for t in ws16] != [(3 * C, C), (C, C), (hidden, C), (C, hidden)]:
+        raise ValueError("vit_tail16: weight shapes do not match the embedding width")
+    if tuple(ln1.normalized_shape) != (C,) or tuple(ln2.normalized_shape) != (C,):
+        raise ValueError("vit_tail16: LayerNorm width does not match the embedding width")
+    bqkv, bproj, bfc1, bfc2 = _opt(bqkv, "qkv.bias"), _opt(bproj, "proj.bias"), _opt(bfc1, "fc1.bias"), _opt(bfc2, "fc2.bias")
+    lnp = [require_device_f32(t, n) for t, n in ((ln1.weight, "layernorm1.weight"), (ln1.bias, "layernorm1.bias"),
+                                                  (ln2.weight, "layernorm2.weight"), (ln2.bias, "layernorm2.bias"))]
+    y = torch.empty(B, C, dtype=torch.float32, device=x.device)
+    nws = lib().mi355_vit_tail_workspace_bytes(B, N, C, hidden)
+    ws = _ffi.workspace_named("mhsa", nws, x.device)
+    check(lib().mi355_vit_tail_fwd(dptr(x), dptr(lnp[0]), dptr(lnp[1]), float(ln1.eps), dptr(ws16[0]), dptr(bqkv), dptr(ws16[1]), dptr(bproj),
+                                   dptr(lnp[2]), dptr(lnp[3]), float(ln2.eps), dptr(ws16[2]), dptr(bfc1), dptr(ws16[3]), dptr(bfc2), dptr(y),
+                                   B, N, C, hidden, int(num_heads), float(scale), p, dptr(ws), nws, stream_ptr(x.device)),
+          "mi355_vit_tail_fwd")
+    return y
+
+
 def logit_envelope(C, K, num_heads, n_tokens):
     return C % num_heads == 0 and C // num_heads in (32, 64) and n_tokens <= 224 and K % 64 == 0 and C % 64 == 0
 
diff --git a/pytorch-attention_amd/mi355attn/modules/vit.py b/pytorch-attention_amd/mi355attn/modules/vit.py
--- a/pytorch-attention_amd/mi355attn/modules/vit.py
+++ b/pytorch-attention_amd/mi355attn/modules/vit.py
@@ -192,6 +192,24 @@
             nn.init.zeros_(m.bias)
             nn.init.ones_(m.weight)
 
+    def _tail_ok(self, blk, tok):
+        if self.global_pool != "token" or F.ln_fold_enabled() or not F.vit_tail_enabled():
+            return False
+        if type(blk) is not TransformerEncoder or type(blk.attn) is not Attention or type(blk.mlp) is not Mlp:
+            return False
+        at, mlp = blk.attn, blk.mlp
+        if F.logit_mode(at.precision) or tok.dim() != 3 or tok.dtype != torch.float32 or not tok.is_cuda:
+            return False
+        p = F._prec(at.precision)
+        B, N, C = tok.shape
+        if p not in (F.PREC_FP16, F.PREC_BF16) or F._prec(mlp.precision) != p or mlp.fc1.in_features != C or mlp.fc2.out_features != C:
+            return False
+        if not (at.fast_ok(N) and _fast(p, mlp.fc1, mlp.fc2) and F.vit_tail_envelope(C, mlp.fc1.out_features, at.num_heads, N)):
+            return False
+        if nn.modules.module._global_forward_hooks or nn.modules.module._global_forward_pre_hooks:
+            return False
+        return not any(m._forward_hooks or m._forward_pre_hooks for m in blk.modules())
+
     def forward(self, x):
         B, _, H, W = x.shape
         ps = self.patch_embedding.patch_size
@@ -200,13 +218,20 @@
                             self.cls_token.reshape(-1), pos, ps, self.precision)
         blocks, state = list(self.blocks), None
         elig = [blk.fold_ok(tok) for blk in blocks] if F.ln_fold_enabled() else None
+        tail = blocks.pop() if blocks and self._tail_ok(blocks[-1], tok) else None
         for i, blk in enumerate(blocks):
             if elig is not None and elig[i]:
                 nxt_ok = i + 1 < len(blocks) and elig[i + 1]
                 tok, state = blk.forward_folded(tok, state, blocks[i + 1].layernorm1.eps if nxt_ok else None)
             else:
                 tok, state = blk(tok), None
-        if self.global_pool == "token":
+        if tail is not None:
+            at, mlp = tail.attn, tail.mlp
+            p = F._prec(at.precision)
+            pooled = F.vit_tail16(tok, tail.layernorm1, F.weight16(at.qkv.weight, p), _bias(at.qkv), F.weight16(at.proj.weight, p),
+                                  at.proj.bias, tail.layernorm2, F.weight16(mlp.fc1.weight, p), mlp.fc1.bias,
+                                  F.weight16(mlp.fc2.weight, p), mlp.fc2.bias, at.num_heads, at.scale, precision=p)
+        elif self.global_pool == "token":
             pooled = tok[:, 0]
         elif self.global_pool == "avg":
             pooled = F.token_mean(tok, skip_first=1)
```

After: 16840 images/s, median of 6. 4.4% higher.
